# BoifZ/VDN-NeRF

Hardware: AMD Instinct MI355X
Metric: rays/sec (512-ray batch, 128 samples/ray) (higher is better)
Workload: dtype bf16; 1 GPU; training step of womsk_white (hierarchical sampling + render forward + backward + gradient all-reduce + Adam): SDF 8x256 + colour 4x256 + NeRF 8x256, 512 rays x (64 coarse + 64 importance + 32 outside) per GPU per step; pixels uniform over the full 800 x 800 frame; samples that enter the loss through exact zeros are skipped: 81 % of the foreground and 56 % of the background points evaluated; rays_per_gpu=512, samples_per_ray=128, outside_samples=32, parallelism=dp1, allreduce_bytes=5636348, background_points_evaluated_last_step=45590, background_points_total=81920, foreground_points_evaluated_last_step=52986, foreground_points_total=65536

## Files before the change

include/vdn_render.h:

```cpp
#ifndef VDN_RENDER_H
#define VDN_RENDER_H
#include <stdint.h>

#ifdef __cplusplus
extern "C" {
#endif

#define VDN_ABI_VERSION 28

int vdn_abi_version(void);

typedef struct {
    const float* g;
    const float* v;
    float* w_eff;
    float* inv_norm;
    int32_t rows, cols;
} VdnWeightNormDesc;
int vdn_weightnorm_materialize(const VdnWeightNormDesc* descs_dev, int n_layers, int max_rows, void* stream);

typedef struct {
    const float* src;
    const float* bias;
    const int32_t* kmap;
    const int32_t* nmap;
    char* dst;
    int64_t row_stride, col_stride;
    int32_t n0;
    int32_t k_pad;
    float scale;
    int32_t fmt;
    int32_t kt_begin;
    int32_t kt_count;
    int32_t write_bias;
    float bias_scale;
    const float* tail;
    int32_t tail_off;
    int32_t tail_n;
    int32_t tail_stride;
} VdnChunkDesc;
int vdn_build_images(const VdnChunkDesc* descs_dev, int n_chunks, void* stream);

int vdn_posenc(const float* in, float* out, int64_t P, int32_t d, int32_t n_freqs, void* stream);

typedef struct {
    const char* blob;
    const float* pts;
    const float* rays_o;
    const float* rays_d;
    const float* z;
    int32_t n_per_ray;
    int32_t z_ld;
    int32_t sdf_ld;
    int32_t P;
    float scale;
    float* sdf;
    void* feat;
    float* normals;
    void* S;
    const float* w8row;
    void* H;
    void* V;
    void* PE;
    const int32_t* active_idx;
    const int32_t* n_active;
    float* U_pe;
    int32_t tail_row0, tail_max_rows;
    int32_t cold_start;
} VdnSdfArgs;
int vdn_sdf_mlp_fwd_f32(int mode, const VdnSdfArgs* args_host, void* stream);
int vdn_sdf_mlp_fwd_bf16(int mode, const VdnSdfArgs* args_host, void* stream);
int vdn_sdf_fwd_tail_bf16(const VdnSdfArgs* args_host, void* stream);

typedef struct {
    const char* blob;
    const float* rays_o;
    const float* rays_d;
    const float* z;
    const float* normals;
    const void* feat;
    const float* pts;
    const float* dirs;
    float* out;
    void* save_h;
    void* save_small;
    int32_t n_per_ray;
    int32_t P;
    int32_t d_out;
    int32_t squeeze_out;
    const int32_t* active_idx;
    const int32_t* n_active;
    const float* extra;
    void* save_extra;
} VdnRenderNetArgs;
int vdn_rendernet_fwd_f32(const VdnRenderNetArgs* args_host, void* stream);
int vdn_rendernet_fwd_bf16(const VdnRenderNetArgs* args_host, void* stream);

typedef struct {
    const char* blob;
    const float* rays_o;
    const float* rays_d;
    const float* z;
    const float* pts4;
    const float* dirs;
    float* density;
    float* rgb;
    float* feat;
    void* save_h;
    void* save_pe;
    void* save_feature;
    void* save_vpe;
    void* save_hv;
    int32_t n_per_ray;
    int32_t P;
    const int32_t* active_idx;
    const int32_t* n_active;
} VdnNerfArgs;
int vdn_nerf_mlp_fwd_f32(const VdnNerfArgs* args_host, void* stream);
int vdn_nerf_mlp_fwd_bf16(const VdnNerfArgs* args_host, void* stream);


typedef struct {
    const float* near;
    const float* far;
    const float* lin_samples;
    const float* lin_outside;
    const float* out_lower;
    const float* out_upper;
    const float* t_rand;
    const float* t_rand_out;
    float* z;
    float* z_out;
    int32_t B, n_samples, n_outside, z_ld;
} VdnCoarseArgs;
int vdn_coarse_z(const VdnCoarseArgs* args_host, void* stream);

typedef struct {
    const float* rays_o;
    const float* rays_d;
    const float* z;
    const float* sdf;
    const float* u;
    float* new_z;
    float inv_s;
    int32_t B, M, ld, n_imp;
    const float* weights;
    int32_t w_ld, _pad;
} VdnUpsampleArgs;
int vdn_upsample_round(const VdnUpsampleArgs* args_host, void* stream);

typedef struct {
    const float* z;
    const float* sdf;
    const float* new_z;
    const float* new_sdf;
    float* z_out;
    float* sdf_out;
    int32_t B, M, K, ld, ld_out;
} VdnMergeArgs;
int vdn_merge_sorted(const VdnMergeArgs* args_host, void* stream);
int vdn_merge_upsample(const VdnMergeArgs* merge_host, const VdnUpsampleArgs* upsample_host, void* stream);
int vdn_sdf_upsample_bf16(const VdnSdfArgs* sdf_host, const VdnUpsampleArgs* upsample_host, void* stream);
int vdn_sdf_merge_upsample_bf16(const VdnSdfArgs* sdf_host, const VdnMergeArgs* merge_host, const VdnUpsampleArgs* upsample_host, void* stream);

typedef struct {
    const float* z;
    float* dists;
    float* mid_z;
    float sample_dist;
    int32_t B, n, ld;
} VdnSectionArgs;
int vdn_sections(const VdnSectionArgs* args_host, void* stream);

typedef struct {
    const float* rays_o;
    const float* rays_d;
    const float* sdf;
    const float* normals;
    const float* dists;
    const float* mid_z;
    const float* color;
    const float* feat;
    const float* variance;
    const float* bg_density;
    const float* bg_rgb;
    const float* bg_feat;
    const float* bg_dists;
    const float* background_rgb;
    float cos_anneal_ratio;
    int32_t B, N, T, feat_ch;
    float* weights;
    float* alpha_out;
    float* cdf;
    float* inside_sphere;
    float* color_out;
    float* feat_out;
    float* weight_sum;
    float* weight_max;
    float* s_val;
    float* eik_partial;
    float* eik_out;
    const float* cos_anneal_dev;
} VdnCompositeArgs;
int vdn_alpha_composite_fwd(const VdnCompositeArgs* args_host, void* stream);
int vdn_feat_composite(const VdnCompositeArgs* args_host, void* stream);

int vdn_shade_fused_f32(const VdnSdfArgs* sdf_host, const VdnRenderNetArgs* color_host, const VdnCompositeArgs* comp_host,
                        int32_t* ticket, void* stream);
int vdn_sdf_color_train_bf16(const VdnSdfArgs* sdf_host, const void* color_blob, int32_t squeeze_out, void* col_h, void* col_small,
                             float* col_out, void* stream);
int vdn_shade_fused_bf16(const VdnSdfArgs* sdf_host, const void* color_blob, int32_t squeeze_out, const VdnCompositeArgs* comp_host,
                         int32_t* ticket, void* stream);

typedef struct {
    const float* rays_o;
    const float* rays_d;
    const float* mid_z;
    const float* normals;
    int32_t B, N;
    float* eik_partial;
    float* eik_out;
} VdnEikonalArgs;
int vdn_eikonal_terms(const VdnEikonalArgs* args_host, void* stream);


typedef struct {
    const char* blob;
    const float* g_out;
    const float* out;
    const void* save_h;
    void* delta_out;
    void* delta_h;
    void* d_feat;
    float* d_normals;
    int32_t acc_feat;
    int32_t acc_normals;
    int32_t P;
    int32_t d_out;
    int32_t squeeze_out;
    const int32_t* active_idx;
    const int32_t* n_active;
    const float* dirs; const float* rays_d;
    int32_t n_per_ray;
    int32_t acc_pts;
    float* d_pts;
    float* d_dirs;
    float* d_extra;
} VdnRenderNetBwdArgs;
int vdn_rendernet_bwd_f32(const VdnRenderNetBwdArgs* args_host, void* stream);
int vdn_rendernet_bwd_bf16(const VdnRenderNetBwdArgs* args_host, void* stream);

typedef struct {
    const char* blob;
    const float* g_density;
    const float* g_rgb;
    const float* g_feat;
    const void* save_h;
    const void* save_hv;
    void* delta_o;
    void* delta_v;
    void* delta_head;
    void* delta_h;
    int32_t P;
    const int32_t* active_idx;
    const int32_t* n_active;
    const float* rays_o; const float* rays_d; const float* z;
    int32_t n_per_ray;
    float* d_pts;
    float* d_dirs;
} VdnNerfBwdArgs;
int vdn_nerf_mlp_bwd_f32(const VdnNerfBwdArgs* args_host, void* stream);
int vdn_nerf_mlp_bwd_bf16(const VdnNerfBwdArgs* args_host, void* stream);
typedef struct {
    const float* pts4;
    const float* dirs;
    float* d_pts4;
    float* d_dirs;
    int32_t accumulate;
} VdnNerfInputGradArgs;
int vdn_nerf_mlp_bwd_input_f32(const VdnNerfBwdArgs* args_host, const VdnNerfInputGradArgs* in_host, void* stream);
int vdn_nerf_mlp_bwd_input_bf16(const VdnNerfBwdArgs* args_host, const VdnNerfInputGradArgs* in_host, void* stream);

typedef struct {
    const char* blob;
    const float* pts;
    const float* rays_o;
    const float* rays_d;
    const float* z;
    int32_t n_per_ray;
    int32_t z_ld;
    int32_t P;
    float scale;
    const float* g_normals;
    const void* S;
    const void* V;
    void* UB;
    void* EX;
    int32_t s_from_h;
    const int32_t* active_idx;
    const int32_t* n_active;
} VdnSdfRbarArgs;
int vdn_sdf_bwd_rbar_f32(const VdnSdfRbarArgs* args_host, void* stream);
int vdn_sdf_bwd_rbar_bf16(const VdnSdfRbarArgs* args_host, void* stream);

typedef struct {
    const char* blob;
    const float* g_sdf;
    const void* g_feat;
    const void* S;
    const void* EX;
    void* AB;
    int32_t P;
    float scale;
    int32_t s_from_h;
    const int32_t* active_idx;
    const int32_t* n_active;
    const float* pts; const float* rays_o; const float* rays_d; const float* z;
    int32_t n_per_ray, z_ld;
    const float* g_normals;
    const float* U_pe;
    int32_t acc_pts;
    float* d_pts;
} VdnSdfFbarArgs;
int vdn_sdf_bwd_fbar_f32(const VdnSdfFbarArgs* args_host, void* stream);
int vdn_sdf_bwd_fbar_bf16(const VdnSdfFbarArgs* args_host, void* stream);
int vdn_sdf_bwd_split_bf16(const VdnSdfRbarArgs* rbar_host, const VdnSdfFbarArgs* fbar_host, void* stream);


typedef struct {
    const void* A1; const void* B1;
    const void* A2; const void* B2;
    int32_t lda1, ldb1, lda2, ldb2;
    int32_t P;
    int32_t m_tiles, n_tiles;
    int32_t splits;
    int32_t wg_begin;
    int32_t _pad;
    float* slab;
    float* colsum;
    const int32_t* P_dev;
} VdnDwDesc;
int vdn_dw_gemm_f32(const VdnDwDesc* descs_dev, int n_desc, int total_wgs, void* stream);
int vdn_dw_gemm_bf16(const VdnDwDesc* descs_dev, int n_desc, int total_wgs, void* stream);
int vdn_dw_entry_wgs_f32(int m_tiles, int n_tiles, int splits);
int vdn_dw_entry_wgs_bf16(int m_tiles, int n_tiles, int splits);

typedef struct {
    const float* slab; const float* colsum;
    const int32_t* rmap; const int32_t* cmap;
    float* target; float* btarget;
    int64_t t_stride;
    int32_t splits, M, N;
    int32_t accumulate;
    float scale, bscale;
    const float* xsum;
    int32_t xsplits, xM, xrow;
    float xscale;
} VdnDwFinalizeDesc;
int vdn_dw_finalize(const VdnDwFinalizeDesc* descs_dev, int n_desc, int max_M, int phase, void* stream);

typedef struct {
    const float* g; const float* v; const float* inv_norm; const float* dw_eff;
    float* dg; float* dv;
    int32_t rows, cols;
} VdnWeightNormBwdDesc;
int vdn_weightnorm_bwd(const VdnWeightNormBwdDesc* descs_dev, int n_layers, int max_rows, void* stream);

typedef struct {
    const float* rays_o; const float* rays_d;
    const float* sdf; const float* normals; const float* dists; const float* mid_z;
    const float* color; const float* feat; const float* variance;
    const float* bg_density; const float* bg_rgb; const float* bg_feat; const float* bg_dists;
    const float* background_rgb;
    float cos_anneal_ratio;
    int32_t B, N, T, feat_ch;
    const float* alpha;
    const float* weights;
    const float* eik;
    const float* g_color;
    const float* g_feat;
    const float* g_weights;
    const float* g_eik;
    const float* g_cdf;
    float* d_sdf;
    float* d_normals;
    float* d_color;
    float* d_feat;
    float* d_bg_density;
    float* d_bg_rgb;
    float* d_bg_feat;
    float* d_var_partial;
    float* d_variance;
    float* d_dists;
    float* d_bg_dists;
    float* d_dir_cos;
    float* feat_scratch;
    const float* cos_anneal_dev;
} VdnCompositeBwdArgs;
int vdn_alpha_composite_bwd(const VdnCompositeBwdArgs* args_host, void* stream);

int vdn_composite_train(const VdnCompositeArgs* fwd_host, const VdnCompositeBwdArgs* bwd_host, const float* true_rgb, float* g_color,
                        const int32_t* fg_count, float igr_weight, float grad_scale, void* stream);
int vdn_eikonal_reduce(const float* eik_partial, int32_t B, float* eik_out, void* stream);
int vdn_composite_fwd_train(const VdnCompositeArgs* fwd_host, const float* gt_feats, float* g_feats, float depth_weight, float grad_scale, void* stream);
int vdn_composite_bwd_train(const VdnCompositeBwdArgs* bwd_host, const float* color_out, const float* true_rgb, float* g_color,
                            const int32_t* fg_count, float igr_weight, float grad_scale, void* stream);

typedef struct {
    const float* rays_d;
    const float* mid_z;
    const float* bg_mid;
    const float* d_pts;
    const float* d_dirs;
    const float* d_dists;
    const float* d_dir_cos;
    const float* d_bg_pts;
    const float* d_bg_dirs;
    const float* d_bg_dists;
    int32_t B, N, T;
    float* d_rays_o;
    float* d_rays_d;
    float* d_z;
    float* d_z_out;
} VdnRayAdjointArgs;
int vdn_ray_adjoint(const VdnRayAdjointArgs* args_host, void* stream);

typedef struct {
    const float* color;
    const float* true_rgb;
    const float* mask;
    const float* feats;
    const float* gt_feats;
    const float* weights;
    const float* eik;
    float igr_weight, mask_weight, depth_weight, grad_scale;
    int32_t B, T, C, _pad;
    float* g_color;
    float* g_feats;
    float* g_weights;
    float* g_eik;
    float* out_scalars;
} VdnLossArgs;
int vdn_loss_fwd_bwd(const VdnLossArgs* args_host, void* stream);

int vdn_adam_step(float* param, const float* grad, float* exp_avg, float* exp_avg_sq, int64_t n,
                  float lr, float beta1, float beta2, float eps, int32_t step, void* stream);
int vdn_adam_step_ranges(float* param, const float* grad, float* exp_avg, float* exp_avg_sq, int64_t begin0, int64_t end0,
                         int64_t begin1, int64_t end1, float lr, float beta1, float beta2, float eps, int32_t step, void* stream);

typedef struct {
    const float* pixels_x;
    const float* pixels_y;
    const float* intrinsic_inv;
    const float* pose;
    const float* image;
    const float* mask;
    const float* feats;
    float* out;
    float* near;
    float* far;
    int32_t B, H, W, C, mask_ch, out_ld;
} VdnGenRaysArgs;
int vdn_gen_rays(const VdnGenRaysArgs* args_host, void* stream);

typedef struct {
    const float* rays_o;
    const float* rays_d;
    const float* mid_z;
    int32_t B, N, T;
    int32_t* active_idx;
    int32_t* n_active;
    int32_t* ray_counts;
} VdnBackgroundActiveArgs;
int vdn_background_active(const VdnBackgroundActiveArgs* args_host, void* stream);

typedef struct {
    const float* rays_o;
    const float* rays_d;
    const float* mid_z;
    int32_t B, N;
    float radius;
    int32_t complement;
    int32_t* active_idx;
    int32_t* n_active;
    int32_t* ray_counts;
} VdnForegroundActiveArgs;

typedef struct {
    const float* rays_o; const float* rays_d;
    float* z;
    const float* new_z;
    int32_t M_old, _pad;
    const float* z_out;
    float* z_feed;
    int32_t B, N, T, z_ld;
    float sample_dist, fg_radius;
    float* dists; float* mid_z;
    float* bg_dists; float* bg_mid;
    int32_t* fg_active_idx; int32_t* fg_n_active; int32_t* fg_ray_counts;
    int32_t* bg_active_idx; int32_t* bg_n_active; int32_t* bg_ray_counts;
} VdnTrainPrepArgs;
int vdn_train_prep(const VdnTrainPrepArgs* args_host, void* stream);
int vdn_foreground_active(const VdnForegroundActiveArgs* args_host, void* stream);

typedef struct {
    const float* u;
    float threshold;
    int32_t R;
    int32_t* counts;
    const int64_t* offsets;
    float* tri_pos;
    int64_t* tri_key;
} VdnMeshArgs;
int vdn_mesh_count(const VdnMeshArgs* args_host, void* stream);
int vdn_mesh_emit(const VdnMeshArgs* args_host, void* stream);

typedef struct {
    const float* u;
    double isovalue;
    int32_t R;
    uint8_t* cube_case;
    int32_t* n_verts;
    int32_t* n_tris;
    const int64_t* vert_offsets;
    const int64_t* tri_offsets;
    double* vertices;
    int64_t* triangles;
} VdnMeshMcArgs;
int vdn_mesh_mc_count(const VdnMeshMcArgs* args_host, void* stream);
int vdn_mesh_mc_emit(const VdnMeshMcArgs* args_host, void* stream);


typedef struct {
    const float* pixels_x;
    const float* pixels_y;
    const float* intrinsic_inv;
    const float* r;
    const float* t;
    const float* init_c2w;
    const float* image;
    const float* mask;
    const float* feats;
    float* out;
    float* near;
    float* far;
    int32_t B, H, W, C, mask_ch, out_ld;
} VdnGenRaysPoseArgs;
int vdn_gen_rays_pose(const VdnGenRaysPoseArgs* args_host, void* stream);

typedef struct {
    const float* pixels_x;
    const float* pixels_y;
    const float* intrinsic_inv;
    const float* r;
    const float* t;
    const float* init_c2w;
    const float* d_rays_o;
    const float* d_rays_d;
    const float* d_z;
    const float* lin_samples;
    const float* d_z_out;
    const float* z_out;
    float* grad_r;
    float* grad_t;
    double* scratch;
    int32_t B, N, O, n_samples, n_importance, cam, n_cams, _pad;
} VdnPoseAdjointArgs;
int vdn_pose_adjoint(const VdnPoseAdjointArgs* args_host, void* stream);
#ifdef __cplusplus
}
#endif
#endif
```

vdn-nerf_amd/csrc/k_nerf_bwd.h:

```cpp
#pragma once
#include <type_traits>
#include "mlp_engine.h"
#include "vdn_kernels.h"

namespace vdn {

template <class P, bool DPT, bool EXPL>
__global__ __launch_bounds__(P::kWaves * 64, P::kMinWavesPerEU) void nerf_bwd_kernel(NerfBwdArgs a, NerfInputGradArgs in) {
    using ST = typename P::store_t;
    constexpr int kSlot = P::stride(9);
    extern __shared__ __attribute__((aligned(16))) char smem[];
    WStream<P::kWaves, kSlot> ws;
    const bool want_pts = EXPL || a.d_pts != nullptr;
    ws.init(a.blob, smem, want_pts ? 83 : 80);
    const int lane = ws.lane, c = lane & 31, h = lane >> 5;
    const long n_rows = a.active_idx != nullptr ? (long)*a.n_active : (long)a.P;
    if ((long)blockIdx.x * P::kWaves * 32 >= n_rows) return;
    ws.warm_issue((n_rows + P::kWaves * 32 - 1) / (P::kWaves * 32), 256 * P::kMinWavesPerEU);
    warm_code_issue((std::is_same<P, BF16>::value) ? kWarmCodeNerfBwd : 0, (n_rows + P::kWaves * 32 - 1) / (P::kWaves * 32), 256 * P::kMinWavesPerEU, ws.warm_dump());
    const long p_raw = ((long)blockIdx.x * P::kWaves + ws.wave) * 32 + c;
    const bool ok = p_raw < n_rows;
    const long p = ok ? p_raw : n_rows - 1;
    const long pd = a.active_idx != nullptr ? (long)a.active_idx[p] : p;
    const long PS = P::plane(a.P, 256);
    constexpr int KO = DPT ? 4 : 1;
    constexpr int LDO = DPT ? 128 : 32;
    const ST* save_h = reinterpret_cast<const ST*>(a.save_h);
    const ST* save_hv = reinterpret_cast<const ST*>(a.save_hv);
    ST* delta_o = reinterpret_cast<ST*>(a.delta_o);
    ST* delta_v = reinterpret_cast<ST*>(a.delta_v);
    ST* delta_head = reinterpret_cast<ST*>(a.delta_head);
    ST* delta_h = reinterpret_cast<ST*>(a.delta_h);

    float x4[4] = {0.0f, 0.0f, 0.0f, 0.0f}, dir[3] = {0.0f, 0.0f, 0.0f}, pw[3] = {0.0f, 0.0f, 0.0f}, nrm = 1.0f;
    float dx4[4] = {0.0f, 0.0f, 0.0f, 0.0f}, ddir[3] = {0.0f, 0.0f, 0.0f};
    if (EXPL) {
#pragma unroll
        for (int d = 0; d < 4; ++d) x4[d] = in.pts4[pd * 4 + d];
#pragma unroll
        for (int d = 0; d < 3; ++d) dir[d] = in.dirs[pd * 3 + d];
    } else if (want_pts) {
        const long r = pd / a.n_per_ray;
        const float z = a.z[pd];
#pragma unroll
        for (int d = 0; d < 3; ++d) {
            dir[d] = a.rays_d[r * 3 + d];
            pw[d] = a.rays_o[r * 3 + d] + dir[d] * z;
        }
        nrm = sqrtf(pw[0] * pw[0] + pw[1] * pw[1] + pw[2] * pw[2]);
        const float rr = fminf(fmaxf(nrm, 1.0f), 1e10f);
#pragma unroll
        for (int d = 0; d < 3; ++d) x4[d] = pw[d] / rr;
        x4[3] = 1.0f / rr;
    }
    typename P::template Act<9> X;
    typename P::template Act<8> Y;
    {
        float g3[3];
#pragma unroll
        for (int d = 0; d < 3; ++d) g3[d] = a.g_rgb[pd * 3 + d];
        const f32x16 t16 = vals_tile<3>(g3, h, 0);
        X.set(0, t16);
        P::store_tile(delta_o, p, LDO, 0, h, t16, ok);
        if constexpr (DPT) {
#pragma unroll
            for (int kt = 0; kt < 3; ++kt) {
                const f32x16 g = F32::load_tile(a.g_feat, pd, 96, kt, h);
                X.set(kt + 1, g);
                P::store_tile(delta_o, p, LDO, kt + 1, h, g, ok);
            }
        }
    }
    auto ldH = [&](int l) VDN_INL { return [=](int nt) VDN_INL { return P::load_tile(save_h + l * PS, p, 256, nt, h); }; };
    auto mask_store = [&](auto& D, ST* dst, int ld) VDN_INL {
        return [&D, dst, ld, p, ok, h](int nt, const f32x16& acc, const f32x16& hv) VDN_INL {
            f32x16 o;
#pragma unroll
            for (int t = 0; t < 16; ++t) o[t] = hv[t] > 0.0f ? acc[t] : 0.0f;
            D.set(nt, o);
            P::store_tile(dst, p, ld, nt, h, o, ok);
        };
    };
    ws.all_issue = __any(ok);
    warm_l2_wait();
    ws.start();
    dense<P, KO, 4, false>(ws, X, 0, [&](int nt) VDN_INL { return P::load_tile(save_hv, p, 128, nt, h); },
                               mask_store(Y, delta_v, 128), 4);
    dense<P, 4, 9, false>(ws, Y, 0, NoPre{}, [&](int nt, const f32x16& acc, int) VDN_INL {
        if (nt < 8) {
            X.set(nt, acc);
            P::store_tile(delta_head, p, 288, nt, h, acc, ok);
        } else if (want_pts) {
            pe_adjoint_tile<3, 4, 0, P::kAccurateTrig>(acc, h, dir, ddir);
        }
    });
    {
        float g1[1] = {a.g_density[pd]};
        const f32x16 t16 = vals_tile<1>(g1, h, 0);
        X.set(8, t16);
        P::store_tile(delta_head, p, 288, 8, h, t16, ok);
    }
    dense<P, 9, 8, false, kBwdPrefetch>(ws, X, 0, ldH(7), mask_store(Y, delta_h + 7 * PS, 256), P::kTileOps, P::kTileOps);
    dense<P, 8, 8, false, kBwdPrefetch>(ws, Y, 0, ldH(6), mask_store(X, delta_h + 6 * PS, 256), P::kTileOps, P::kTileOps);
    dense<P, 8, 8, false, kBwdPrefetch>(ws, X, 0, ldH(5), mask_store(Y, delta_h + 5 * PS, 256), P::kTileOps, P::kTileOps);
    dense<P, 8, 11, false>(ws, Y, 0,
        [&](int nt) VDN_INL { return nt >= 3 ? P::load_tile(save_h + 4 * PS, p, 256, nt - 3, h) : f32x16{}; },
        [&](int nt, const f32x16& acc, const f32x16& hv) VDN_INL {
            if (nt >= 3) {
                f32x16 o;
#pragma unroll
                for (int t = 0; t < 16; ++t) o[t] = hv[t] > 0.0f ? acc[t] : 0.0f;
                X.set(nt - 3, o);
                P::store_tile(delta_h + 4 * PS, p, 256, nt - 3, h, o, ok);
            } else if (want_pts) {
                if (nt == 0) pe_adjoint_tile<4, 10, 0, P::kAccurateTrig>(acc, h, x4, dx4);
                else if (nt == 1) pe_adjoint_tile<4, 10, 1, P::kAccurateTrig>(acc, h, x4, dx4);
                else pe_adjoint_tile<4, 10, 2, P::kAccurateTrig>(acc, h, x4, dx4);
            }
        });
    dense<P, 8, 8, false, kBwdPrefetch>(ws, X, 0, ldH(3), mask_store(Y, delta_h + 3 * PS, 256), P::kTileOps, P::kTileOps);
    dense<P, 8, 8, false, kBwdPrefetch>(ws, Y, 0, ldH(2), mask_store(X, delta_h + 2 * PS, 256), P::kTileOps, P::kTileOps);
    dense<P, 8, 8, false, kBwdPrefetch>(ws, X, 0, ldH(1), mask_store(Y, delta_h + 1 * PS, 256), P::kTileOps, P::kTileOps);
    dense<P, 8, 8, false, kBwdPrefetch>(ws, Y, 0, ldH(0), mask_store(X, delta_h + 0 * PS, 256), P::kTileOps, P::kTileOps);
    if (want_pts) {
        dense<P, 8, 3, false>(ws, X, 0, NoPre{}, [&](int nt, const f32x16& acc, int) VDN_INL {
            if (nt == 0) pe_adjoint_tile<4, 10, 0, P::kAccurateTrig>(acc, h, x4, dx4);
            else if (nt == 1) pe_adjoint_tile<4, 10, 1, P::kAccurateTrig>(acc, h, x4, dx4);
            else pe_adjoint_tile<4, 10, 2, P::kAccurateTrig>(acc, h, x4, dx4);
        });
        if (EXPL) {
            if (ok && h == 0) {
#pragma unroll
                for (int d = 0; d < 4; ++d) in.d_pts4[pd * 4 + d] = (in.accumulate ? in.d_pts4[pd * 4 + d] : 0.0f) + dx4[d];
#pragma unroll
                for (int d = 0; d < 3; ++d) in.d_dirs[pd * 3 + d] = (in.accumulate ? in.d_dirs[pd * 3 + d] : 0.0f) + ddir[d];
            }
            return;
        }
        if (ok && h == 0) {
            const bool free_r = nrm >= 1.0f && nrm <= 1e10f;
            const float rr = fminf(fmaxf(nrm, 1.0f), 1e10f);
            const float pu = pw[0] * dx4[0] + pw[1] * dx4[1] + pw[2] * dx4[2];
#pragma unroll
            for (int d = 0; d < 3; ++d) {
                float v = dx4[d] / rr;
                if (free_r) v -= pw[d] * (pu / (rr * rr * rr) + dx4[3] / (rr * rr * rr));
                a.d_pts[pd * 3 + d] = v;
                a.d_dirs[pd * 3 + d] = ddir[d];
            }
        }
    }
}

template <class P, bool EXPL>
int launch_nerf_bwd_impl(const VdnNerfBwdArgs* args, const NerfInputGradArgs& in, void* stream_) {
    hipStream_t stream = (hipStream_t)stream_;
    const int ppw = P::kWaves * 32;
    const int grid = (args->P + ppw - 1) / ppw;
    const size_t lds = 3 * P::stride(9);
    static bool once = (allow_big_lds(nerf_bwd_kernel<P, false, EXPL>, lds), allow_big_lds(nerf_bwd_kernel<P, true, EXPL>, lds), true);
    (void)once;
    if (args->g_feat != nullptr)
        hipLaunchKernelGGL((nerf_bwd_kernel<P, true, EXPL>), dim3(grid), dim3(P::kWaves * 64), lds, stream, *args, in);
    else
        hipLaunchKernelGGL((nerf_bwd_kernel<P, false, EXPL>), dim3(grid), dim3(P::kWaves * 64), lds, stream, *args, in);
    return (int)hipGetLastError();
}

inline bool nerf_bwd_args_ok(const VdnNerfBwdArgs* args) {
    return args && args->P > 0 && args->blob && args->g_density && args->g_rgb && args->save_h && args->save_hv &&
           args->delta_o && args->delta_v && args->delta_head && args->delta_h;
}

template <class P>
int launch_nerf_bwd(const VdnNerfBwdArgs* args, void* stream) {
    if (!nerf_bwd_args_ok(args)) return -1;
    if (args->d_pts && (!args->d_dirs || !args->rays_o || !args->rays_d || !args->z || args->n_per_ray <= 0)) return -2;
    return launch_nerf_bwd_impl<P, false>(args, NerfInputGradArgs{}, stream);
}

template <class P>
int launch_nerf_bwd_input(const VdnNerfBwdArgs* args, const VdnNerfInputGradArgs* in, void* stream) {
    if (!nerf_bwd_args_ok(args)) return -1;
    if (!in || !in->pts4 || !in->dirs || !in->d_pts4 || !in->d_dirs) return -2;
    if (args->d_pts || args->d_dirs) return -3;
    return launch_nerf_bwd_impl<P, true>(args, *in, stream);
}

}
```

vdn-nerf_amd/csrc/k_nerf_fwd.h:

```cpp
#pragma once
#include "mlp_engine.h"
#include "vdn_kernels.h"

namespace vdn {

template <class P, bool DPT>
__global__ __launch_bounds__(P::kWaves * 64, P::kMinWavesPerEU) void nerf_fwd_kernel(NerfArgs a) {
    using ST = typename P::store_t;
    constexpr int kSlot = P::stride(11);
    extern __shared__ __attribute__((aligned(16))) char smem[];
    WStream<P::kWaves, kSlot> ws;
    ws.init(a.blob, smem, 64 + 9 + 4 + (DPT ? 4 : 1));
    const int lane = ws.lane, c = lane & 31, h = lane >> 5;
    const long n_rows = a.active_idx != nullptr ? (long)*a.n_active : (long)a.P;
    if ((long)blockIdx.x * P::kWaves * 32 >= n_rows) return;
    if (a.save_h != nullptr) ws.warm((n_rows + P::kWaves * 32 - 1) / (P::kWaves * 32), 256 * P::kMinWavesPerEU);
    const long q_raw = ((long)blockIdx.x * P::kWaves + ws.wave) * 32 + c;
    const bool ok = q_raw < n_rows;
    const long q = ok ? q_raw : n_rows - 1;
    const long p = a.active_idx != nullptr ? (long)a.active_idx[q] : q;
    const long r = p / a.n_per_ray;
    ST* save_h = reinterpret_cast<ST*>(a.save_h);
    const long PS = P::plane(a.P, 256);

    float dir[3], p4[4];
#pragma unroll
    for (int d = 0; d < 3; ++d) dir[d] = a.dirs ? a.dirs[p * 3 + d] : a.rays_d[r * 3 + d];
    if (a.pts4 != nullptr) {
#pragma unroll
        for (int d = 0; d < 4; ++d) p4[d] = a.pts4[p * 4 + d];
    } else {
        const float z = a.z[p];
        float q[3];
        float n2 = 0.0f;
#pragma unroll
        for (int d = 0; d < 3; ++d) {
            q[d] = a.rays_o[r * 3 + d] + a.rays_d[r * 3 + d] * z;
            n2 += q[d] * q[d];
        }
        const float rr = fminf(fmaxf(sqrtf(n2), 1.0f), 1e10f);
#pragma unroll
        for (int d = 0; d < 3; ++d) p4[d] = q[d] / rr;
        p4[3] = 1.0f / rr;
    }
    typename P::template Act<11> X;
    typename P::template Act<9> Y;
    auto put_pe = [&](bool save) VDN_INL {
        float pe[84];
        posenc<4, 10, P::kAccurateTrig>(p4, pe);
#pragma unroll
        for (int kt = 0; kt < 3; ++kt) {
            const f32x16 t16 = vals_tile<84>(pe, h, kt);
            X.set(kt, t16);
            if (save && a.save_pe != nullptr) P::store_tile(reinterpret_cast<ST*>(a.save_pe), q, 96, kt, h, t16, ok);
        }
    };
    auto relu_into = [&](auto& D, int t0, ST* save, int ld) VDN_INL {
        return [&D, t0, save, ld, q, ok, h](int nt, const f32x16& acc, int) VDN_INL {
            f32x16 o;
#pragma unroll
            for (int t = 0; t < 16; ++t) o[t] = relu0(acc[t]);
            D.set(t0 + nt, o);
            if (save != nullptr) P::store_tile(save, q, ld, nt, h, o, ok);
        };
    };
    auto sv = [&](int l) VDN_INL { return save_h ? save_h + l * PS : (ST*)nullptr; };
    const int est = save_h != nullptr ? P::kTileOps : 0;
    ws.all_issue = __any(ok);
    put_pe(true);
    ws.start();
    dense<P, 3, 8, true>(ws, X, 0, NoPre{}, relu_into(Y, 0, sv(0), 256), est);
    dense<P, 8, 8, true>(ws, Y, 0, NoPre{}, relu_into(X, 0, sv(1), 256), est);
    dense<P, 8, 8, true>(ws, X, 0, NoPre{}, relu_into(Y, 0, sv(2), 256), est);
    dense<P, 8, 8, true>(ws, Y, 0, NoPre{}, relu_into(X, 0, sv(3), 256), est);
    dense<P, 8, 8, true>(ws, X, 0, NoPre{}, relu_into(Y, 0, sv(4), 256), est);
#pragma unroll
    for (int kt = 0; kt < 8; ++kt) X.copy_tile(3 + kt, Y, kt);
    put_pe(false);
    dense<P, 11, 8, true>(ws, X, 0, NoPre{}, relu_into(Y, 0, sv(5), 256), est);
    dense<P, 8, 8, true>(ws, Y, 0, NoPre{}, relu_into(X, 0, sv(6), 256), est);
    dense<P, 8, 8, true>(ws, X, 0, NoPre{}, relu_into(Y, 0, sv(7), 256), est);
    dense<P, 8, 9, true>(ws, Y, 0, NoPre{}, [&](int nt, const f32x16& acc, int) VDN_INL {
        if (nt < 8) {
            X.set(nt, acc);
            if (a.save_feature != nullptr) P::store_tile(reinterpret_cast<ST*>(a.save_feature), q, 256, nt, h, acc, ok);
        } else {
            if (ok && h == 0) a.density[p] = acc[0];
        }
    });
    {
        float pe[27];
        posenc<3, 4, P::kAccurateTrig>(dir, pe);
        const f32x16 t16 = vals_tile<27>(pe, h, 0);
        X.set(8, t16);
        if (a.save_vpe != nullptr) P::store_tile(reinterpret_cast<ST*>(a.save_vpe), q, 32, 0, h, t16, ok);
    }
    dense<P, 9, 4, true>(ws, X, 0, NoPre{}, relu_into(Y, 0, reinterpret_cast<ST*>(a.save_hv), 128));
    dense<P, 4, DPT ? 4 : 1, true>(ws, Y, 0, NoPre{}, [&](int nt, const f32x16& acc, int) VDN_INL {
        if (nt == 0) {
            if (ok && h == 0) {
                a.rgb[p * 3 + 0] = acc[0];
                a.rgb[p * 3 + 1] = acc[1];
                a.rgb[p * 3 + 2] = acc[2];
            }
        } else {
            F32::store_tile(a.feat, p, 96, nt - 1, h, acc, ok);
        }
    });
}

template <class P>
int launch_nerf_fwd(const VdnNerfArgs* args, void* stream_) {
    hipStream_t stream = (hipStream_t)stream_;
    if (args == nullptr || args->P <= 0 || !args->blob || !args->density || !args->rgb || args->n_per_ray <= 0) return -1;
    if (!args->pts4 && (!args->rays_o || !args->rays_d || !args->z)) return -1;
    if (!args->dirs && !args->rays_d) return -1;
    const int ppw = P::kWaves * 32;
    const int grid = (args->P + ppw - 1) / ppw;
    const size_t lds = 3 * P::stride(11);
    static bool once = (allow_big_lds(nerf_fwd_kernel<P, false>, lds), allow_big_lds(nerf_fwd_kernel<P, true>, lds), true);
    (void)once;
    if (args->feat != nullptr)
        hipLaunchKernelGGL((nerf_fwd_kernel<P, true>), dim3(grid), dim3(P::kWaves * 64), lds, stream, *args);
    else
        hipLaunchKernelGGL((nerf_fwd_kernel<P, false>), dim3(grid), dim3(P::kWaves * 64), lds, stream, *args);
    return (int)hipGetLastError();
}

}
```

vdn-nerf_amd/csrc/k_nerf_fwd2.h:

```cpp
#pragma once
#include "mlp_flow.h"
#include "vdn_kernels.h"

namespace vdn {

template <bool DPT, bool SAVE>
struct NerfFwdProg {
    static constexpr int total = 64 + 9 + 4 + (DPT ? 4 : 1);
    static constexpr int kt(int c) {
        if (c < 0 || c >= total) return 0;
        if (c < 8) return 3;
        if (c < 40) return 8;
        if (c < 48) return 11;
        if (c < 73) return 8;
        if (c < 77) return 9;
        return 4;
    }
    static constexpr bool bias(int c) { return c >= 0 && c < total; }
    static constexpr int loads(int) { return 0; }
    static constexpr bool drained(int c) { return c == 39; }
    static constexpr int stores(int c) {
        if (!SAVE || c < 0 || c >= total) return 0;
        if (c < 64) return BF16::kTileOps;
        if (c < 72) return BF16::kTileOps;
        if (c < 73) return 0;
        if (c < 77) return BF16::kTileOps;
        return 0;
    }
};

#ifndef VDN_NERF_FWD_ST_MODE
#define VDN_NERF_FWD_ST_MODE VDN_PLANE_ST_MODE
#endif
template <bool DPT, bool SAVE>
__global__ __launch_bounds__(256, 2) void nerf_fwd2_kernel(NerfArgs a) {
    constexpr int kSt = VDN_NERF_FWD_ST_MODE;
    using P = BF16;
    using ST = unsigned short;
    using PG = NerfFwdProg<DPT, SAVE>;
    constexpr int kSlot = P::stride(11);
    extern __shared__ __attribute__((aligned(16))) char smem[];
    flow::Pipe<4, kSlot, 3, 2> pp;
    pp.init(a.blob, smem);
    const int lane = pp.lane, c = lane & 31, h = lane >> 5;
    const long n_rows = a.active_idx != nullptr ? (long)*a.n_active : (long)a.P;
    if ((long)blockIdx.x * 4 * 32 >= n_rows) return;
    char* const wdump = pp.warm_dump();
    if constexpr (SAVE) warm_l2_issue(a.blob, PG::total * kSlot, (n_rows + 127) / 128, 512, wdump);
    warm_code_issue(SAVE ? kWarmCodeNerfFwd2 : 0, (n_rows + 127) / 128, 512, wdump);
    const long q_raw = ((long)blockIdx.x * 4 + pp.wave) * 32 + c;
    const bool ok = q_raw < n_rows;
    const long q = ok ? q_raw : n_rows - 1;
    const long p = a.active_idx != nullptr ? (long)a.active_idx[q] : q;
    const long r = p / a.n_per_ray;
    ST* save_h = reinterpret_cast<ST*>(a.save_h);
    const long PS = P::plane(a.P, 256);

    float dir[3], p4[4];
#pragma unroll
    for (int d = 0; d < 3; ++d) dir[d] = a.dirs ? a.dirs[p * 3 + d] : a.rays_d[r * 3 + d];
    if (a.pts4 != nullptr) {
#pragma unroll
        for (int d = 0; d < 4; ++d) p4[d] = a.pts4[p * 4 + d];
    } else {
        const float z = a.z[p];
        float qq[3];
        float n2 = 0.0f;
#pragma unroll
        for (int d = 0; d < 3; ++d) {
            qq[d] = a.rays_o[r * 3 + d] + a.rays_d[r * 3 + d] * z;
            n2 += qq[d] * qq[d];
        }
        const float rr = fminf(fmaxf(sqrtf(n2), 1.0f), 1e10f);
#pragma unroll
        for (int d = 0; d < 3; ++d) p4[d] = qq[d] / rr;
        p4[3] = 1.0f / rr;
    }
    typename P::template Act<11> X;
    typename P::template Act<9> Y;
    bf16x8 pe_keep[6];
    {
        float pe[84];
        posenc<4, 10, false>(p4, pe);
#pragma unroll
        for (int kt = 0; kt < 3; ++kt) {
            const f32x16 t16 = vals_tile<84>(pe, h, kt);
            X.set(kt, t16);
            if constexpr (SAVE) {
                if (a.save_pe != nullptr) P::template store_tile<kSt>(reinterpret_cast<ST*>(a.save_pe), q, 96, kt, h, t16, true);
            }
        }
#pragma unroll
        for (int i = 0; i < 6; ++i) pe_keep[i] = X.r[i];
    }
    auto relu_into = [&](auto& D, int t0, ST* save, int ld) VDN_INL {
        return [&D, t0, save, ld, q, h](int nt, const f32x16& acc, int) VDN_INL {
            f32x16 o;
#pragma unroll
            for (int t = 0; t < 16; ++t) o[t] = relu0(acc[t]);
            D.set(t0 + nt, o);
            if constexpr (SAVE) P::template store_tile<kSt>(save, q, ld, nt, h, o, true);
        };
    };
    auto sv = [&](int l) VDN_INL { return save_h + l * PS; };
    warm_l2_wait();
    pp.template start<PG>();
    auto f0 = flow::flow_begin();
    auto f1 = flow::dense2<PG, 8>(f0, pp, X, flow::NoLoad{}, relu_into(Y, 0, sv(0), 256));
    auto f2 = flow::dense2<PG, 8>(f1, pp, Y, flow::NoLoad{}, relu_into(X, 0, sv(1), 256));
    auto f3 = flow::dense2<PG, 8>(f2, pp, X, flow::NoLoad{}, relu_into(Y, 0, sv(2), 256));
    auto f4 = flow::dense2<PG, 8>(f3, pp, Y, flow::NoLoad{}, relu_into(X, 0, sv(3), 256));
    auto f5 = flow::dense2<PG, 8>(f4, pp, X, flow::NoLoad{}, relu_into(Y, 0, sv(4), 256));
    auto f5d = flow::flow_drain(f5);
#pragma unroll
    for (int kt = 0; kt < 8; ++kt) X.copy_tile(3 + kt, Y, kt);
#pragma unroll
    for (int i = 0; i < 6; ++i) X.r[i] = pe_keep[i];
    auto f6 = flow::dense2<PG, 8>(f5d, pp, X, flow::NoLoad{}, relu_into(Y, 0, sv(5), 256));
    auto f7 = flow::dense2<PG, 8>(f6, pp, Y, flow::NoLoad{}, relu_into(X, 0, sv(6), 256));
    auto f8 = flow::dense2<PG, 8>(f7, pp, X, flow::NoLoad{}, relu_into(Y, 0, sv(7), 256));
    auto f9 = flow::dense2<PG, 9>(f8, pp, Y, flow::NoLoad{}, [&](int nt, const f32x16& acc, int) VDN_INL {
        if (nt < 8) {
            X.set(nt, acc);
            if constexpr (SAVE) {
                if (a.save_feature != nullptr) P::template store_tile<kSt>(reinterpret_cast<ST*>(a.save_feature), q, 256, nt, h, acc, true);
            }
        } else {
            if (ok && h == 0) a.density[p] = acc[0];
        }
    });
    {
        float pe[27];
        posenc<3, 4, false>(dir, pe);
        const f32x16 t16 = vals_tile<27>(pe, h, 0);
        X.set(8, t16);
        if constexpr (SAVE) {
            if (a.save_vpe != nullptr) P::template store_tile<kSt>(reinterpret_cast<ST*>(a.save_vpe), q, 32, 0, h, t16, true);
        }
    }
    auto f10 = flow::dense2<PG, 4, false>(f9, pp, X, flow::NoLoad{}, relu_into(Y, 0, reinterpret_cast<ST*>(a.save_hv), 128));
    auto f11 = flow::dense2<PG, DPT ? 4 : 1>(f10, pp, Y, flow::NoLoad{}, [&](int nt, const f32x16& acc, int) VDN_INL {
        if (nt == 0) {
            if (ok && h == 0) {
                a.rgb[p * 3 + 0] = acc[0];
                a.rgb[p * 3 + 1] = acc[1];
                a.rgb[p * 3 + 2] = acc[2];
            }
        } else {
            F32::store_tile(a.feat, p, 96, nt - 1, h, acc, ok);
        }
    });
    flow::flow_finish(f11);
}

inline int launch_nerf_fwd2(const VdnNerfArgs* args, void* stream_) {
    hipStream_t stream = (hipStream_t)stream_;
    if (args == nullptr || args->P <= 0 || !args->blob || !args->density || !args->rgb || args->n_per_ray <= 0) return -1;
    if (!args->pts4 && (!args->rays_o || !args->rays_d || !args->z)) return -1;
    if (!args->dirs && !args->rays_d) return -1;
    const bool save = args->save_h != nullptr;
    if (save && (!args->save_hv || !args->save_feature)) return -1;
    const int grid = (args->P + 127) / 128;
    const size_t lds = 3 * BF16::stride(11);
    static bool once = (allow_big_lds(nerf_fwd2_kernel<false, false>, lds), allow_big_lds(nerf_fwd2_kernel<true, false>, lds),
                        allow_big_lds(nerf_fwd2_kernel<false, true>, lds), allow_big_lds(nerf_fwd2_kernel<true, true>, lds), true);
    (void)once;
    const bool dpt = args->feat != nullptr;
#define VDN_L(D, S) hipLaunchKernelGGL((nerf_fwd2_kernel<D, S>), dim3(grid), dim3(256), lds, stream, *args)
    if (dpt) { if (save) VDN_L(true, true); else VDN_L(true, false); }
    else { if (save) VDN_L(false, true); else VDN_L(false, false); }
#undef VDN_L
    return (int)hipGetLastError();
}

}
```

vdn-nerf_amd/csrc/k_render_bwd.h:

```cpp
#pragma once
#include <type_traits>
#include "mlp_engine.h"
#include "vdn_kernels.h"

namespace vdn {

template <class P, int NT_OUT, int EX = 0>
__global__ __launch_bounds__(P::kWaves * 64, P::kMinWavesPerEU) void rendernet_bwd_kernel(RenderNetBwdArgs a) {
    using ST = typename P::store_t;
    constexpr int kSlot = P::stride(8);
    extern __shared__ __attribute__((aligned(16))) char smem[];
    WStream<P::kWaves, kSlot> ws;
    ws.init(a.blob, smem, 42 + EX);
    const int lane = ws.lane, c = lane & 31, h = lane >> 5;
    const WorkRow wr = work_row(a.active_idx, a.n_active, a.P, P::kWaves, ws.wave, c);
    if (wr.none) return;
    ws.warm_issue(wr.n_wg, 256 * P::kMinWavesPerEU);
    warm_code_issue((std::is_same<P, BF16>::value) ? kWarmCodeRenderBwd : 0, wr.n_wg, 256 * P::kMinWavesPerEU, ws.warm_dump());
    const bool ok = wr.ok;
    const long p = wr.row, pd = wr.point;
    const long PS = P::plane(a.P, 256);
    const ST* save_h = reinterpret_cast<const ST*>(a.save_h);
    ST* delta_h = reinterpret_cast<ST*>(a.delta_h);
    ST* delta_out = reinterpret_cast<ST*>(a.delta_out);
    ST* d_feat = reinterpret_cast<ST*>(a.d_feat);

    typename P::template Act<8> X, Y;
    if constexpr (NT_OUT == 1) {
        float dl[4];
#pragma unroll
        for (int j = 0; j < 4; ++j) {
            dl[j] = 0.0f;
            if (j < a.d_out) {
                const float o = a.out[pd * a.d_out + j], g = a.g_out[pd * a.d_out + j];
                dl[j] = a.squeeze_out ? g * o * (1.0f - o) : (o > 0.0f ? g : 0.0f);
            }
        }
        const f32x16 t16 = vals_tile<4>(dl, h, 0);
        X.set(0, t16);
        P::store_tile(delta_out, p, 32, 0, h, t16, ok);
    } else {
#pragma unroll
        for (int kt = 0; kt < 3; ++kt) {
            const f32x16 o = F32::load_tile(a.out, pd, 96, kt, h);
            const f32x16 g = F32::load_tile(a.g_out, pd, 96, kt, h);
            f32x16 dl;
#pragma unroll
            for (int t = 0; t < 16; ++t) dl[t] = a.squeeze_out ? g[t] * o[t] * (1.0f - o[t]) : (o[t] > 0.0f ? g[t] : 0.0f);
            X.set(kt, dl);
            P::store_tile(delta_out, p, 96, kt, h, dl, ok);
        }
    }
    auto ldH = [&](int l) VDN_INL { return [=](int nt) VDN_INL { return P::load_tile(save_h + l * PS, p, 256, nt, h); }; };
    auto mask_store = [&](auto& D, int l) VDN_INL {
        return [&D, l, delta_h, PS, p, ok, h](int nt, const f32x16& acc, const f32x16& hv) VDN_INL {
            f32x16 o;
#pragma unroll
            for (int t = 0; t < 16; ++t) o[t] = hv[t] > 0.0f ? acc[t] : 0.0f;
            D.set(nt, o);
            P::store_tile(delta_h + l * PS, p, 256, nt, h, o, ok);
        };
    };
    ws.all_issue = __any(ok);
    warm_l2_wait();
    ws.start();
    dense<P, NT_OUT, 8, false, kBwdPrefetch>(ws, X, 0, ldH(3), mask_store(Y, 3), P::kTileOps, P::kTileOps);
    dense<P, 8, 8, false, kBwdPrefetch>(ws, Y, 0, ldH(2), mask_store(X, 2), P::kTileOps, P::kTileOps);
    dense<P, 8, 8, false, kBwdPrefetch>(ws, X, 0, ldH(1), mask_store(Y, 1), P::kTileOps, P::kTileOps);
    dense<P, 8, 8, false, kBwdPrefetch>(ws, Y, 0, ldH(0), mask_store(X, 0), P::kTileOps, P::kTileOps);
    f32x16 SM[2];
    dense<P, 8, 10 + EX, false>(ws, X, 0, NoPre{}, [&](int nt, const f32x16& acc, int) VDN_INL {
        if (nt >= 10) {
            if constexpr (EX > 0) {
                f32x16 o = F32::load_tile(a.d_extra, pd, 32 * EX, nt - 10, h);
#pragma unroll
                for (int t = 0; t < 16; ++t) o[t] += acc[t];
                F32::store_tile(a.d_extra, pd, 32 * EX, nt - 10, h, o, ok);
            }
        } else if (nt < 8) {
            f32x16 o = acc;
            if (a.acc_feat) {
                const f32x16 prev = P::load_tile(d_feat, p, 256, nt, h);
#pragma unroll
                for (int t = 0; t < 16; ++t) o[t] += prev[t];
            }
            P::store_tile(d_feat, p, 256, nt, h, o, ok);
        } else {
            SM[nt - 8] = acc;
        }
    });
    float small[33];
    tiles_vals<33, 2>(SM, h, small);
    if (ok && h == 0) {
#pragma unroll
        for (int d = 0; d < 3; ++d) {
            const float prev = a.acc_normals ? a.d_normals[pd * 3 + d] : 0.0f;
            a.d_normals[pd * 3 + d] = prev + small[30 + d];
        }
        if (a.d_pts != nullptr) {
            const long r = pd / a.n_per_ray;
#pragma unroll
            for (int d = 0; d < 3; ++d) {
                const float dir = a.dirs ? a.dirs[pd * 3 + d] : a.rays_d[r * 3 + d];
                float g = small[3 + d];
#pragma unroll
                for (int k = 0; k < 4; ++k) {
                    const float f = (float)(1 << k);
                    float sn, co;
                    sincos_pe<P::kAccurateTrig>(dir * f, sn, co);
                    g += f * (co * small[3 + 3 + 6 * k + d] - sn * small[3 + 3 + 6 * k + 3 + d]);
                }
                const float pp = a.acc_pts ? a.d_pts[pd * 3 + d] : 0.0f;
                const float pg = a.acc_pts ? a.d_dirs[pd * 3 + d] : 0.0f;
                a.d_pts[pd * 3 + d] = pp + small[d];
                a.d_dirs[pd * 3 + d] = pg + g;
            }
        }
    }
}

template <class P>
int launch_rendernet_bwd(const VdnRenderNetBwdArgs* args, void* stream_) {
    hipStream_t stream = (hipStream_t)stream_;
    if (!args || args->P <= 0 || !args->blob || !args->g_out || !args->out || !args->save_h || !args->delta_out ||
        !args->delta_h || !args->d_feat || !args->d_normals) return -1;
    if (!(args->d_out == 96 || (args->d_out >= 1 && args->d_out <= 4))) return -2;
    if (args->d_pts && (!args->d_dirs || (!args->dirs && (!args->rays_d || args->n_per_ray <= 0)))) return -3;
    const int ppw = P::kWaves * 32;
    const int grid = (args->P + ppw - 1) / ppw;
    const size_t lds = 3 * P::stride(8);
    static bool once = (allow_big_lds(rendernet_bwd_kernel<P, 1>, lds), allow_big_lds(rendernet_bwd_kernel<P, 3>, lds),
                        allow_big_lds(rendernet_bwd_kernel<P, 1, 3>, lds), true);
    (void)once;
    if (args->d_extra != nullptr) {
        if (args->d_out == 96) return -4;
        hipLaunchKernelGGL((rendernet_bwd_kernel<P, 1, 3>), dim3(grid), dim3(P::kWaves * 64), lds, stream, *args);
        return (int)hipGetLastError();
    }
    if (args->d_out == 96)
        hipLaunchKernelGGL((rendernet_bwd_kernel<P, 3>), dim3(grid), dim3(P::kWaves * 64), lds, stream, *args);
    else
        hipLaunchKernelGGL((rendernet_bwd_kernel<P, 1>), dim3(grid), dim3(P::kWaves * 64), lds, stream, *args);
    return (int)hipGetLastError();
}

}
```

vdn-nerf_amd/csrc/k_render_fwd.h:

```cpp
#pragma once
#include <type_traits>
#include "mlp_engine.h"
#include "vdn_kernels.h"

namespace vdn {

template <class P, int NT_OUT, int EX = 0>
VDN_DEV void rendernet_fwd_body(const RenderNetArgs& a, char* smem) {
    using ST = typename P::store_t;
    constexpr int kSlot = P::stride(10 + EX);
    constexpr int kNSlot = 3 * kSlot > 160 * 1024 ? 2 : 3;
    WStream<P::kWaves, kSlot, kNSlot> ws;
    ws.init(a.blob, smem, 32 + NT_OUT);
    const int lane = ws.lane, c = lane & 31, h = lane >> 5;
    const WorkRow wr = work_row(a.active_idx, a.n_active, a.P, P::kWaves, ws.wave, c);
    if (wr.none) return;
    if (a.save_h != nullptr) ws.warm_issue(wr.n_wg, 256 * P::kMinWavesPerEU);
    warm_code_issue((a.save_h != nullptr && std::is_same<P, BF16>::value) ? kWarmCodeRenderFwd : 0, wr.n_wg, 256 * P::kMinWavesPerEU, ws.warm_dump());
    const bool ok = wr.ok;
    const long p = wr.row, pd = wr.point;
    const long r = pd / a.n_per_ray;
    const ST* feat = reinterpret_cast<const ST*>(a.feat);
    ST* save_h = reinterpret_cast<ST*>(a.save_h);
    ST* save_small = reinterpret_cast<ST*>(a.save_small);
    const long PS = P::plane(a.P, 256);

    typename P::template Act<10 + EX> X;
    typename P::template Act<8> Y;
#pragma unroll
    for (int kt = 0; kt < 8; ++kt) X.set(kt, P::load_tile(feat, p, 256, kt, h));
    if constexpr (EX > 0) {
#pragma unroll
        for (int kt = 0; kt < EX; ++kt) {
            const f32x16 t16 = F32::load_tile(a.extra, pd, 32 * EX, kt, h);
            X.set(10 + kt, t16);
            if (a.save_extra != nullptr) P::store_tile(reinterpret_cast<ST*>(a.save_extra), p, 32 * EX, kt, h, t16, ok);
        }
    }
    {
        float small[33];
        float dir[3];
        const float z = a.pts ? 0.0f : a.z[pd];
#pragma unroll
        for (int d = 0; d < 3; ++d) {
            dir[d] = a.dirs ? a.dirs[pd * 3 + d] : a.rays_d[r * 3 + d];
            small[d] = a.pts ? a.pts[pd * 3 + d] : a.rays_o[r * 3 + d] + a.rays_d[r * 3 + d] * z;
            small[30 + d] = a.normals[pd * 3 + d];
        }
        float pe[27];
        posenc<3, 4, P::kAccurateTrig>(dir, pe);
#pragma unroll
        for (int i = 0; i < 27; ++i) small[3 + i] = pe[i];
#pragma unroll
        for (int kt = 0; kt < 2; ++kt) {
            const f32x16 t16 = vals_tile<33>(small, h, kt);
            X.set(8 + kt, t16);
            if (save_small != nullptr) P::store_tile(save_small, p, 64, kt, h, t16, ok);
        }
    }
    auto relu_into = [&](auto& D, int l) VDN_INL {
        return [&D, l, save_h, PS, p, ok, h](int nt, const f32x16& acc, int) VDN_INL {
            f32x16 o;
#pragma unroll
            for (int t = 0; t < 16; ++t) o[t] = relu0(acc[t]);
            D.set(nt, o);
            if (save_h != nullptr) P::store_tile(save_h + l * PS, p, 256, nt, h, o, ok);
        };
    };
    const int est = save_h != nullptr ? P::kTileOps : 0;
    ws.all_issue = __any(ok);
    warm_l2_wait();
    ws.start();
    dense<P, 10 + EX, 8, true>(ws, X, 0, NoPre{}, relu_into(Y, 0), est);
    dense<P, 8, 8, true>(ws, Y, 0, NoPre{}, relu_into(X, 1), est);
    dense<P, 8, 8, true>(ws, X, 0, NoPre{}, relu_into(Y, 2), est);
    dense<P, 8, 8, true>(ws, Y, 0, NoPre{}, relu_into(X, 3), est);
    dense<P, 8, NT_OUT, true>(ws, X, 0, NoPre{}, [&](int nt, const f32x16& acc, int) VDN_INL {
        f32x16 o;
#pragma unroll
        for (int t = 0; t < 16; ++t) o[t] = a.squeeze_out ? sigmoidf_(acc[t]) : relu0(acc[t]);
        if constexpr (NT_OUT == 1) {
            if (ok && h == 0) {
                for (int j = 0; j < a.d_out && j < 4; ++j) a.out[pd * a.d_out + j] = o[j];
            }
        } else {
            F32::store_tile(a.out, pd, 96, nt, h, o, ok);
        }
    });
}

template <class P, int NT_OUT, int EX = 0>
__global__ __launch_bounds__(P::kWaves * 64, P::kMinWavesPerEU) void rendernet_fwd_kernel(RenderNetArgs a) {
    extern __shared__ __attribute__((aligned(16))) char smem[];
    rendernet_fwd_body<P, NT_OUT, EX>(a, smem);
}

template <class P>
int launch_rendernet_fwd(const VdnRenderNetArgs* args, void* stream_) {
    hipStream_t stream = (hipStream_t)stream_;
    if (args == nullptr || args->P <= 0 || !args->blob || !args->normals || !args->feat || !args->out || args->n_per_ray <= 0) return -1;
    if (!args->pts && (!args->rays_o || !args->rays_d || !args->z)) return -1;
    if (!args->dirs && !args->rays_d) return -1;
    if (!(args->d_out == 96 || (args->d_out >= 1 && args->d_out <= 4))) return -2;
    const int ppw = P::kWaves * 32;
    const int grid = (args->P + ppw - 1) / ppw;
    if (args->extra != nullptr) {
        if (args->d_out == 96) return -3;
        const size_t lds3 = (3 * P::stride(13) > 160 * 1024 ? 2 : 3) * P::stride(13);
        static bool once3 = (allow_big_lds(rendernet_fwd_kernel<P, 1, 3>, lds3), true);
        (void)once3;
        hipLaunchKernelGGL((rendernet_fwd_kernel<P, 1, 3>), dim3(grid), dim3(P::kWaves * 64), lds3, stream, *args);
        return (int)hipGetLastError();
    }
    const size_t lds = 3 * P::stride(10);
    static bool once = (allow_big_lds(rendernet_fwd_kernel<P, 1>, lds), allow_big_lds(rendernet_fwd_kernel<P, 3>, lds), true);
    (void)once;
    if (args->d_out == 96)
        hipLaunchKernelGGL((rendernet_fwd_kernel<P, 3>), dim3(grid), dim3(P::kWaves * 64), lds, stream, *args);
    else
        hipLaunchKernelGGL((rendernet_fwd_kernel<P, 1>), dim3(grid), dim3(P::kWaves * 64), lds, stream, *args);
    return (int)hipGetLastError();
}

}
```

vdn-nerf_amd/csrc/mlp_engine.h:

```cpp
#pragma once
#include <type_traits>
#include "vdn_common.h"

namespace vdn {

typedef __bf16 bf16x2_t __attribute__((ext_vector_type(2)));

VDN_DEV unsigned pack_bf16x2(float a, float b) {
    bf16x2_t v = {(__bf16)a, (__bf16)b};
    return __builtin_bit_cast(unsigned, v);
}
VDN_DEV float bf16_lo(unsigned u) { return __uint_as_float(u << 16); }
VDN_DEV float bf16_hi(unsigned u) { return __uint_as_float(u & 0xFFFF0000u); }


template <int NWAVES, int STRIDE, int NSLOT = 3>
struct WStream {
    static_assert(STRIDE % (1024 * NWAVES) == 0, "chunk stride must be a multiple of NWAVES KiB");
    static constexpr int DEPTH = NSLOT - 1;
    static constexpr int G = STRIDE / 1024 / NWAVES;
    const char* g;
    char* lds;
    int cur;
    int issued;
    int total;
    int wave, lane;
    bool all_issue;

    unsigned voff0, m0_wave;
    VDN_DEV void init(const char* blob, char* smem, int total_chunks) {
        g = blob;
        lds = smem;
        cur = -1;
        issued = 0;
        total = total_chunks;
        wave = threadIdx.x >> 6;
        lane = threadIdx.x & 63;
        all_issue = false;
        const int wv = __builtin_amdgcn_readfirstlane(wave);
        voff0 = lane * 16 + wv * (G * 1024) + 4096;
        m0_wave = __builtin_amdgcn_readfirstlane((unsigned)(size_t)smem + wv * (G * 1024) + 4096);
    }
    VDN_DEV char* warm_dump() const { return lds + (threadIdx.x >> 6) * (G * 1024); }
    VDN_DEV void warm(long n_wg, int resident) const { warm_l2(g, total * STRIDE, n_wg, resident, warm_dump()); }
    VDN_DEV void warm_issue(long n_wg, int resident) const { warm_l2_issue(g, total * STRIDE, n_wg, resident, warm_dump()); }
    VDN_DEV void issue_next() {
        const unsigned m0v = m0_wave + (unsigned)((issued % NSLOT) * STRIDE);
        static_for<G>([&](auto i_c) VDN_INL {
            constexpr int I = decltype(i_c)::value;
            if constexpr (I % 8 == 0) glds16_imm_m0<glds_imm(I)>(g, voff0 + glds_group_off(I), m0v + glds_group_off(I));
            else glds16_imm<glds_imm(I)>(g, voff0 + glds_group_off(I));
        });
        g += STRIDE;
        ++issued;
    }
    VDN_DEV void start() {
#pragma unroll
        for (int i = 0; i < DEPTH; ++i)
            if (issued < total) issue_next();
    }
    VDN_DEV const char* acquire(int younger = 0) {
        ++cur;
        if (!all_issue) younger = 0;
        const int ahead = min(issued - cur - 1, DEPTH - 1);
        wait_vm(younger + ahead * G);
#if !defined(VDN_ABLATE) || VDN_ABLATE != 3
        __builtin_amdgcn_s_barrier();
#endif
        asm volatile("" ::: "memory");
        if (issued < total) issue_next();
        return lds + (cur % NSLOT) * STRIDE;
    }
    static VDN_DEV void wait_vm(int n) {
        switch (n) {
#define VDN_W(k) case k: asm volatile("s_waitcnt vmcnt(" #k ")" ::: "memory"); break;
            VDN_W(1) VDN_W(2) VDN_W(3) VDN_W(4) VDN_W(5) VDN_W(6) VDN_W(7) VDN_W(8) VDN_W(9) VDN_W(10) VDN_W(11) VDN_W(12)
            VDN_W(13) VDN_W(14) VDN_W(15) VDN_W(16) VDN_W(17) VDN_W(18) VDN_W(19) VDN_W(20) VDN_W(21) VDN_W(22) VDN_W(23) VDN_W(24)
            VDN_W(25) VDN_W(26) VDN_W(27) VDN_W(28) VDN_W(29) VDN_W(30) VDN_W(31) VDN_W(32)
#undef VDN_W
            default: if (n > 32) { asm volatile("s_waitcnt vmcnt(32)" ::: "memory"); } else { asm volatile("s_waitcnt vmcnt(0)" ::: "memory"); } break;
        }
    }
};

VDN_DEV float sprime(float raw, int from_h) {
    if (from_h == 0) return raw;
    return 1.0f - __builtin_amdgcn_exp2f(from_h == 2 ? -raw : -144.26950408889634f * raw);
}

struct WorkRow {
    long row, point;
    bool ok, none;
    long n_wg;
};
VDN_DEV WorkRow work_row(const int32_t* active_idx, const int32_t* n_active, long P, int waves, int wave, int c) {
    WorkRow w;
    const long n_rows = active_idx != nullptr ? (long)*n_active : P;
    w.none = (long)blockIdx.x * waves * 32 >= n_rows;
    const long raw = ((long)blockIdx.x * waves + wave) * 32 + c;
    w.ok = raw < n_rows;
    w.row = w.ok ? raw : (n_rows > 0 ? n_rows - 1 : 0);
    w.point = active_idx != nullptr ? (long)active_idx[w.row] : w.row;
    w.n_wg = (n_rows + waves * 32 - 1) / (waves * 32);
    return w;
}

struct NoPre {
    VDN_DEV int operator()(int) const { return 0; }
};

struct F32 {
    static constexpr int kWaves = 4;
    static constexpr int kMinWavesPerEU = 1;
    static constexpr bool kAccurateTrig = true;
    static constexpr bool kOverlapEpilogue = false;
    static constexpr bool kDeriveS = false;
    static constexpr int chunk_bytes(int KT) { return KT * 4096 + 1024; }
    static constexpr int stride(int KTMAX) { return (chunk_bytes(KTMAX) + 4095) / 4096 * 4096; }
    static constexpr int kTileOps = 4;
    using store_t = float;

    template <int NT>
    struct Act {
        float r[NT * 16];
        VDN_DEV void set(int tile, const f32x16& v) {
#pragma unroll
            for (int t = 0; t < 16; ++t) {
                float x = v[t];
                asm volatile("" : "+v"(x));
                r[tile * 16 + t] = x;
            }
        }
        template <class A2>
        VDN_DEV void copy_tile(int dt, const A2& src, int st) {
#pragma unroll
            for (int t = 0; t < 16; ++t) r[dt * 16 + t] = src.r[st * 16 + t];
        }
    };

    template <int KT, bool BIAS, class ActT>
    static VDN_DEV f32x16 mma(const char* w, const ActT& X, int x0, int lane) {
        const int h = lane >> 5;
        const f32x4* wa = reinterpret_cast<const f32x4*>(w) + lane;
        f32x16 acc;
        if constexpr (BIAS) {
            const f32x4* bias = reinterpret_cast<const f32x4*>(w + KT * 4096);
#pragma unroll
            for (int q = 0; q < 4; ++q) {
                const f32x4 b = bias[2 * q + h];
                acc[4 * q + 0] = b[0]; acc[4 * q + 1] = b[1]; acc[4 * q + 2] = b[2]; acc[4 * q + 3] = b[3];
            }
        } else {
#pragma unroll
            for (int t = 0; t < 16; ++t) acc[t] = 0.0f;
        }
        static_for<KT * 4>([&](auto g_c) VDN_INL {
            constexpr int g = decltype(g_c)::value;
            const f32x4 a = wa[g * 64];
            acc = __builtin_amdgcn_mfma_f32_32x32x2f32(a[0], X.r[x0 * 16 + 4 * g + 0], acc, 0, 0, 0);
            acc = __builtin_amdgcn_mfma_f32_32x32x2f32(a[1], X.r[x0 * 16 + 4 * g + 1], acc, 0, 0, 0);
            acc = __builtin_amdgcn_mfma_f32_32x32x2f32(a[2], X.r[x0 * 16 + 4 * g + 2], acc, 0, 0, 0);
            acc = __builtin_amdgcn_mfma_f32_32x32x2f32(a[3], X.r[x0 * 16 + 4 * g + 3], acc, 0, 0, 0);
        });
        return acc;
    }

    static VDN_DEV long plane(long P, int ld) { return P * ld; }
    static VDN_DEV long rows(long P) { return P; }
    static VDN_DEV void store_tile(float* base, long row, int ld, int tile, int h, const f32x16& v, bool ok) {
        if (!ok) return;
        float* p = base + row * ld + tile * 32 + 4 * h;
#pragma unroll
        for (int q = 0; q < 4; ++q) {
            f32x4 o = {v[4 * q], v[4 * q + 1], v[4 * q + 2], v[4 * q + 3]};
            *reinterpret_cast<f32x4*>(p + 8 * q) = o;
        }
    }
    using raw_tile = f32x16;
    static VDN_DEV raw_tile load_raw(const float* base, long row, int ld, int tile, int h) { return load_tile(base, row, ld, tile, h); }
    static VDN_DEV f32x16 unpack(const raw_tile& r) { return r; }
    static VDN_DEV f32x16 load_tile(const float* base, long row, int ld, int tile, int h) {
        const float* p = base + row * ld + tile * 32 + 4 * h;
        f32x16 r;
#pragma unroll
        for (int q = 0; q < 4; ++q) {
            const f32x4 o = *reinterpret_cast<const f32x4*>(p + 8 * q);
            r[4 * q] = o[0]; r[4 * q + 1] = o[1]; r[4 * q + 2] = o[2]; r[4 * q + 3] = o[3];
        }
        return r;
    }
};

struct BF16 {
    static constexpr int kWaves = 4;
    static constexpr int kMinWavesPerEU = 2;
    static constexpr bool kAccurateTrig = false;
    static constexpr bool kOverlapEpilogue = true;
    static constexpr bool kDeriveS = true;
#ifndef VDN_SLOT_GROUP
#define VDN_SLOT_GROUP 2
#endif
    static constexpr int kSlotGroup = VDN_SLOT_GROUP;
    static constexpr int chunk_bytes(int KT) { return KT * 2048 + 1024; }
    static constexpr int stride(int KTMAX) { return (chunk_bytes(KTMAX) + 4095) / 4096 * 4096; }
    using store_t = unsigned short;

    template <int NT>
    struct Act {
        bf16x8 r[NT * 2];
        VDN_DEV void set(int tile, const f32x16& v) {
#pragma unroll
            for (int s = 0; s < 2; ++s) {
                typedef unsigned u32x4 __attribute__((ext_vector_type(4)));
                u32x4 pk;
#pragma unroll
                for (int j = 0; j < 4; ++j) {
                    unsigned x = pack_bf16x2(v[8 * s + 2 * j], v[8 * s + 2 * j + 1]);
                    asm volatile("" : "+v"(x));
                    pk[j] = x;
                }
                r[tile * 2 + s] = __builtin_bit_cast(bf16x8, pk);
            }
        }
        template <class A2>
        VDN_DEV void copy_tile(int dt, const A2& src, int st) {
            r[dt * 2] = src.r[st * 2];
            r[dt * 2 + 1] = src.r[st * 2 + 1];
        }
    };

    template <int KT, bool BIAS, class ActT>
    static VDN_DEV f32x16 mma(const char* w, const ActT& X, int x0, int lane) {
        const int h = lane >> 5;
        const bf16x8* wa = reinterpret_cast<const bf16x8*>(w) + lane;
        f32x16 acc;
        if constexpr (BIAS) {
            const f32x4* bias = reinterpret_cast<const f32x4*>(w + KT * 2048);
#pragma unroll
            for (int q = 0; q < 4; ++q) {
                const f32x4 b = bias[2 * q + h];
                acc[4 * q + 0] = b[0]; acc[4 * q + 1] = b[1]; acc[4 * q + 2] = b[2]; acc[4 * q + 3] = b[3];
            }
        } else {
#pragma unroll
            for (int t = 0; t < 16; ++t) acc[t] = 0.0f;
        }
#if defined(VDN_ABLATE) && VDN_ABLATE == 2
        (void)wa;
        return acc;
#endif
        constexpr int NS = KT * 2;
        constexpr int PRE = NS < 6 ? NS : 6;
        bf16x8 fr[NS];
        static_for<NS>([&](auto s_c) VDN_INL {
            constexpr int s = decltype(s_c)::value;
            fr[s] = wa[s * 64];
        });
        static_for<NS>([&](auto s_c) VDN_INL {
            constexpr int s = decltype(s_c)::value;
            acc = __builtin_amdgcn_mfma_f32_32x32x16_bf16(fr[s], X.r[x0 * 2 + s], acc, 0, 0, 0);
        });
        __builtin_amdgcn_sched_group_barrier(0x100, PRE + (BIAS ? 2 : 0), 0);
        static_for<NS - PRE>([&](auto) VDN_INL {
            __builtin_amdgcn_sched_group_barrier(0x008, 1, 0);
            __builtin_amdgcn_sched_group_barrier(0x100, 1, 0);
        });
        __builtin_amdgcn_sched_group_barrier(0x008, PRE, 0);
        return acc;
    }

    template <int KT, bool BIAS, class ActT, class Slot>
    static VDN_DEV f32x16 mma_slots(const char* w, const ActT& X, int x0, int lane, Slot&& slot) {
        const int h = lane >> 5;
        const bf16x8* wa = reinterpret_cast<const bf16x8*>(w) + lane;
        constexpr int NS = KT * 2;
        constexpr int PRE = NS < 6 ? NS : 6;
        f32x16 acc;
        bf16x8 fr[NS];
        static_for<PRE>([&](auto s_c) VDN_INL {
            constexpr int s = decltype(s_c)::value;
            fr[s] = wa[s * 64];
        });
        if constexpr (BIAS) {
            const f32x4* bias = reinterpret_cast<const f32x4*>(w + KT * 2048);
#pragma unroll
            for (int q = 0; q < 4; ++q) {
                const f32x4 b = bias[2 * q + h];
                acc[4 * q + 0] = b[0]; acc[4 * q + 1] = b[1]; acc[4 * q + 2] = b[2]; acc[4 * q + 3] = b[3];
            }
        } else {
#pragma unroll
            for (int t = 0; t < 16; ++t) acc[t] = 0.0f;
        }
        __builtin_amdgcn_sched_barrier(0);
        static_for<NS>([&](auto s_c) VDN_INL {
            constexpr int s = decltype(s_c)::value;
            acc = __builtin_amdgcn_mfma_f32_32x32x16_bf16(fr[s], X.r[x0 * 2 + s], acc, 0, 0, 0);
            if constexpr (s + PRE < NS) fr[s + PRE] = wa[(s + PRE) * 64];
            slot(s_c, std::integral_constant<int, NS>{});
            if constexpr ((s + 1) % kSlotGroup == 0 || s + 1 == NS) __builtin_amdgcn_sched_barrier(0);
        });
        return acc;
    }

    static constexpr int kTileOps = 2;
    static VDN_DEV long rows(long P) { return (P + 31) & ~31L; }
    static VDN_DEV long plane(long P, int ld) { return rows(P) * ld; }
    template <int MODE = VDN_PLANE_ST_MODE>
    static VDN_DEV void store_tile(unsigned short* base, long row, int ld, int tile, int h, const f32x16& v, bool ok) {
        if (!ok) return;
        unsigned short* p = base + (row >> 5) * (32L * ld) + tile * 1024 + h * 256 + (row & 31) * 8;
#pragma unroll
        for (int k = 0; k < 2; ++k) {
            uint4 o;
            o.x = pack_bf16x2(v[8 * k], v[8 * k + 1]);
            o.y = pack_bf16x2(v[8 * k + 2], v[8 * k + 3]);
            o.z = pack_bf16x2(v[8 * k + 4], v[8 * k + 5]);
            o.w = pack_bf16x2(v[8 * k + 6], v[8 * k + 7]);
            typedef unsigned wt_u32x4 __attribute__((ext_vector_type(4)));
            const wt_u32x4 ov = {o.x, o.y, o.z, o.w};
            if constexpr (MODE == 1) asm volatile("global_store_dwordx4 %0, %1, off sc1\n\ts_nop 1" ::"v"(p + 512 * k), "v"(ov) : "memory");
            else if constexpr (MODE == 2) asm volatile("global_store_dwordx4 %0, %1, off nt\n\ts_nop 1" ::"v"(p + 512 * k), "v"(ov) : "memory");
            else if constexpr (MODE == 3) asm volatile("global_store_dwordx4 %0, %1, off sc1 nt\n\ts_nop 1" ::"v"(p + 512 * k), "v"(ov) : "memory");
            else if constexpr (MODE == 4) { asm volatile("" ::"v"(p + 512 * k), "v"(ov)); }
            else *reinterpret_cast<uint4*>(p + 512 * k) = o;
        }
    }
    struct raw_tile { uint4 k[2]; };
    static VDN_DEV raw_tile load_raw(const unsigned short* base, long row, int ld, int tile, int h) {
        const unsigned short* p = base + (row >> 5) * (32L * ld) + tile * 1024 + h * 256 + (row & 31) * 8;
        raw_tile r;
#ifdef VDN_PLANE_LD_NT
        typedef unsigned nt_u32x4 __attribute__((ext_vector_type(4)));
        const nt_u32x4 a = __builtin_nontemporal_load(reinterpret_cast<const nt_u32x4*>(p));
        const nt_u32x4 b = __builtin_nontemporal_load(reinterpret_cast<const nt_u32x4*>(p + 512));
        r.k[0] = make_uint4(a[0], a[1], a[2], a[3]);
        r.k[1] = make_uint4(b[0], b[1], b[2], b[3]);
#else
        r.k[0] = *reinterpret_cast<const uint4*>(p);
        r.k[1] = *reinterpret_cast<const uint4*>(p + 512);
#endif
        return r;
    }
    static VDN_DEV f32x16 unpack(const raw_tile& t) {
        f32x16 r;
#pragma unroll
        for (int k = 0; k < 2; ++k) {
            const uint4 o = t.k[k];
            r[8 * k] = bf16_lo(o.x); r[8 * k + 1] = bf16_hi(o.x); r[8 * k + 2] = bf16_lo(o.y); r[8 * k + 3] = bf16_hi(o.y);
            r[8 * k + 4] = bf16_lo(o.z); r[8 * k + 5] = bf16_hi(o.z); r[8 * k + 6] = bf16_lo(o.w); r[8 * k + 7] = bf16_hi(o.w);
        }
        return r;
    }
    static VDN_DEV f32x16 load_tile(const unsigned short* base, long row, int ld, int tile, int h) {
        return unpack(load_raw(base, row, ld, tile, h));
    }
};

template <class ScratchT, class Elem, class Finish>
struct ElemEpi {
    using Scratch = ScratchT;
    Elem elem;
    Finish finish;
    template <class Aux>
    VDN_DEV void operator()(int nt, const f32x16& acc, const Aux& aux) const {
        Scratch sc;
#pragma unroll
        for (int t = 0; t < 16; ++t) elem(nt, t, acc[t], sc);
        finish(nt, sc, aux);
    }
};
template <class ScratchT, class Elem, class Finish>
VDN_DEV ElemEpi<ScratchT, Elem, Finish> elem_epi(Elem e, Finish f) { return {e, f}; }
template <class T> struct is_elem_epi : std::false_type {};
template <class S, class E, class F> struct is_elem_epi<ElemEpi<S, E, F>> : std::true_type {};

template <class P, int KT, int NT, bool BIAS, int PF = 1, class WS, class ActT, class Pre, class Epi>
VDN_DEV void dense(WS& ws, const ActT& X, int x0, Pre&& pre, Epi&& epi, int epi_stores = 0, int pre_loads = 0) {
    const int lane = ws.lane;
    using EpiT = std::remove_cv_t<std::remove_reference_t<Epi>>;
    if constexpr (P::kOverlapEpilogue && is_elem_epi<EpiT>::value) {
        f32x16 acc_prev;
        decltype(pre(0)) aux_prev{};
        static_for<NT + 1>([&](auto s_c) VDN_INL {
            constexpr int s = decltype(s_c)::value;
            typename EpiT::Scratch sc;
            if constexpr (s < NT) {
                constexpr int D = WS::DEPTH;
                constexpr int n_pre = s < D ? s : D;
                constexpr int n_epi = s <= D ? (s > 0 ? s - 1 : 0) : D;
                const int yg = n_pre * pre_loads + n_epi * epi_stores;
                const char* w = ws.acquire(yg);
                auto aux_cur = pre(s);
                const f32x16 acc_cur = P::template mma_slots<KT, BIAS>(w, X, x0, lane, [&](auto k_c, auto ns_c) VDN_INL {
                    if constexpr (s > 0) {
                        constexpr int k = decltype(k_c)::value, NS = decltype(ns_c)::value;
                        static_for<(k + 1) * 16 / NS - k * 16 / NS>([&](auto j_c) VDN_INL {
                            constexpr int t = k * 16 / NS + decltype(j_c)::value;
                            epi.elem(s - 1, t, acc_prev[t], sc);
                        });
                    }
                });
                if constexpr (s > 0) epi.finish(s - 1, sc, aux_prev);
                acc_prev = acc_cur;
                aux_prev = aux_cur;
            } else {
#pragma unroll
                for (int t = 0; t < 16; ++t) epi.elem(s - 1, t, acc_prev[t], sc);
                epi.finish(s - 1, sc, aux_prev);
            }
            __builtin_amdgcn_sched_barrier(0);
        });
        return;
    }
    using Aux = decltype(pre(0));
    Aux ring[PF];
    static_for<PF>([&](auto i_c) VDN_INL {
        constexpr int i = decltype(i_c)::value;
        if constexpr (i < NT) ring[i] = pre(i);
    });
    static_for<NT>([&](auto nt_c) VDN_INL {
        constexpr int nt = decltype(nt_c)::value;
        constexpr int n_steps = nt < WS::DEPTH ? nt : WS::DEPTH;
        constexpr int n_pre = [] { int n = 0; for (int j = nt - n_steps; j < nt; ++j) n += (j + PF < NT) ? 1 : 0; return n; }();
        const int yg = n_steps * epi_stores + n_pre * pre_loads;
        const char* w = ws.acquire(yg);
        Aux nxt{};
        if constexpr (nt + PF < NT) nxt = pre(nt + PF);
        const f32x16 acc = P::template mma<KT, BIAS>(w, X, x0, lane);
        epi(nt, acc, ring[nt % PF]);
        if constexpr (nt + PF < NT) ring[nt % PF] = nxt;
        __builtin_amdgcn_sched_barrier(0);
    });
}

#ifndef VDN_BWD_PF
#define VDN_BWD_PF 2
#endif
constexpr int kBwdPrefetch = VDN_BWD_PF;

template <int NF>
VDN_DEV f32x16 vals_tile(const float (&vals)[NF], int h, int tile) {
    f32x16 o;
#pragma unroll
    for (int t = 0; t < 16; ++t) {
        const int f0 = 32 * tile + (t & 3) + 8 * (t >> 2);
        const int f1 = f0 + 4;
        const float a = f0 < NF ? vals[f0 < NF ? f0 : 0] : 0.0f;
        const float b = f1 < NF ? vals[f1 < NF ? f1 : 0] : 0.0f;
        o[t] = h ? b : a;
    }
    return o;
}
template <int NF, int NT>
VDN_DEV void tiles_vals(const f32x16 (&T)[NT], int h, float (&vals)[NF]) {
#pragma unroll
    for (int tile = 0; tile < NT; ++tile) {
#pragma unroll
        for (int t = 0; t < 16; ++t) {
            const int f0 = 32 * tile + (t & 3) + 8 * (t >> 2);
            const int f1 = f0 + 4;
            const float mine = T[tile][t];
            const float other = __shfl_xor(mine, 32);
            if (f0 < NF) vals[f0 < NF ? f0 : 0] = h ? other : mine;
            if (f1 < NF) vals[f1 < NF ? f1 : 0] = h ? mine : other;
        }
    }
}

template <int D, int L, int T0, bool ACCURATE>
VDN_DEV void pe_adjoint_tile(const f32x16& tile, int h, const float (&x)[D], float (&dx)[D]) {
    float g[32];
    const f32x16 t1[1] = {tile};
    tiles_vals<32, 1>(t1, h, g);
#pragma unroll
    for (int j = 0; j < 32; ++j) {
        const int slot = 32 * T0 + j;
        if (slot >= D * (1 + 2 * L)) continue;
        if (slot < D) {
            dx[slot] += g[j];
        } else {
            const int k = (slot - D) / (2 * D), w = (slot - D) % (2 * D), d = w % D;
            const float f = (float)(1 << k);
            float sn, co;
            sincos_pe<ACCURATE>(x[d] * f, sn, co);
            dx[d] += w >= D ? -f * sn * g[j] : f * co * g[j];
        }
    }
}

}
```

vdn-nerf_amd/vdn_hip/layout.py:

```python
import torch


def pad32(P):
    return (P + 31) // 32 * 32


def rows(P, precision):
    return P if precision == "fp32" else pad32(P)


def to_pt32(x):
    P, ld = x.shape
    Pp = pad32(P)
    buf = torch.zeros(Pp, ld, dtype=torch.bfloat16, device=x.device)
    buf[:P] = x.to(torch.bfloat16)
    return buf.view(Pp // 32, 32, ld // 32, 2, 2, 2, 4).permute(0, 2, 3, 5, 1, 4, 6).contiguous().view(-1)


def from_pt32(buf, P, ld):
    Pp = pad32(P)
    x = buf.view(-1)[:Pp * ld].view(Pp // 32, ld // 32, 2, 2, 32, 2, 4).permute(0, 4, 1, 2, 5, 3, 6).contiguous().view(Pp, ld)
    return x[:P].float()


def col_offset_elems(col0, precision):
    if precision == "fp32":
        return col0
    assert col0 % 32 == 0
    return (col0 // 32) * 1024
```

vdn-nerf_amd/vdn_hip/train.py:

```python
import os

import numpy as np
import torch

from . import images, layout, lib

PTS_PER_SPLIT = int(os.environ.get("VDN_DW_SPLIT_PTS", "4096"))


def _pts_per_split(net, precision="bf16"):
    if precision == "fp32":
        dflt = "2048"
        return int(os.environ.get("VDN_DW_SPLIT_PTS_SDF" if net == "sdf" else "VDN_DW_SPLIT_PTS_REST", dflt))
    if net == "sdf":
        return int(os.environ.get("VDN_DW_SPLIT_PTS_SDF", os.environ.get("VDN_DW_SPLIT_PTS", "6144")))
    rest = os.environ.get("VDN_DW_SPLIT_PTS_REST", str(PTS_PER_SPLIT))
    return int(os.environ.get("VDN_DW_SPLIT_PTS_NERF" if net == "nerf" else "VDN_DW_SPLIT_PTS_HEADS", rest))


_stream = lib.stream_handle


_SHARED_STREAMS = {}


def shared_stream(dev, role):
    key = (torch.device(dev).index if torch.device(dev).index is not None else torch.cuda.current_device(), role)
    st = _SHARED_STREAMS.get(key)
    if st is None:
        st = _SHARED_STREAMS[key] = torch.cuda.Stream(device=dev)
    return st


class _Net:

    def __init__(self, module, dev, grad_views):
        self.module = module
        self.img = module._images()
        self.dweff = torch.zeros_like(self.img.weff)
        self.grads = {}
        for name, (g, v, b) in self.img.matrices.items():
            for t in (g, v, b):
                if t is not None:
                    self.grads[id(t)] = grad_views[id(t)]

    def dweff_view(self, name):
        v = self.img.matrices[name][1]
        o = self.img.w_off[name]
        return self.dweff[o:o + v.numel()].view(v.shape)

    def dw_target(self, name):
        g, v, b = self.img.matrices[name]
        return self.dweff_view(name) if g is not None else self.grads[id(v)]

    def bias_target(self, name):
        b = self.img.matrices[name][2]
        return None if b is None else self.grads[id(b)]



def _sl(t, l, ld=256):
    return (t, l * t.shape[1] * t.shape[2], 0, ld)


def _whole(t, c0=0):
    return (t, 0, c0, t.shape[1])


def sdf_dw_entries(H, V, PE, UB, AB, P, Pp, precision):
    ub_off, off = {}, 0
    for l, cols in enumerate((64, 256, 256, 256, 288, 256, 256, 256, 256)):
        ub_off[l] = (off, cols)
        off += Pp * cols
    ub = lambda l, c0=0: (UB, ub_off[l][0], c0, ub_off[l][1])
    ab = lambda l: (AB, 0, 0, 288) if l == 8 else (AB, Pp * 288 + (7 - l) * Pp * 256, 0, 256)
    maps = images.sdf_layer_maps()
    unit = 1.0 / images.SDF_UNIT if precision == "bf16" else 1.0
    maps = [(name, km, nm, sc * unit) for (name, km, nm, sc) in maps]
    ent = []
    for l, (name, km, nm, sc) in enumerate(maps):
        if l == 8:
            ent.append(dict(net="sdf", name=name, rmap=nm, cmap=km, scale=sc, A=ab(8), B=_sl(H, 7), bias=True, Pn=P))
            continue
        A, A2 = ab(l), _sl(V, l)
        if l == 0:
            ent.append(dict(net="sdf", name=name, rmap=nm, cmap=km, scale=sc, A=A, B=_whole(PE), A2=A2, B2=ub(0), bias=True, Pn=P))
        elif l == 4:
            ent.append(dict(net="sdf", name=name, rmap=nm, cmap=km[:224], scale=sc, A=A, B=_sl(H, 3), A2=A2, B2=ub(4), bias=True, Pn=P))
            ent.append(dict(net="sdf", name=name, rmap=nm, cmap=km[224:], scale=sc, A=A, B=_whole(PE), A2=A2, B2=ub(4, 224), bias=False, Pn=P))
        else:
            ent.append(dict(net="sdf", name=name, rmap=nm, cmap=km, scale=sc, A=A, B=_sl(H, l - 1), A2=A2, B2=ub(l), bias=True, Pn=P))
    ent.append(dict(net="sdf", name="lin8", rmap=images.ident_map(256), cmap=None, scale=1.0, A=ub(8), B=None, bias=False, Pn=P,
                    extra_row0=True))
    return ent


def rendering_dw_entries(net, km0, dh, dout, save_h, small, feat, extra, P, d_out):
    pad = 96 if d_out == 96 else 32
    I256 = images.ident_map(256)
    ent = [dict(net=net, name="lin0", rmap=I256, cmap=km0[:256], scale=1.0, A=_sl(dh, 0), B=_whole(feat), bias=True, Pn=P),
           dict(net=net, name="lin0", rmap=I256, cmap=km0[256:320], scale=1.0, A=_sl(dh, 0), B=_whole(small), bias=False, Pn=P)]
    if len(km0) > 320:
        ent.append(dict(net=net, name="lin0", rmap=I256, cmap=km0[320:], scale=1.0, A=_sl(dh, 0), B=_whole(extra), bias=False, Pn=P))
    for l in (1, 2, 3):
        ent.append(dict(net=net, name="lin%d" % l, rmap=I256, cmap=I256, scale=1.0, A=_sl(dh, l), B=_sl(save_h, l - 1), bias=True, Pn=P))
    ent.append(dict(net=net, name="lin4", rmap=images.ident_map(d_out, pad), cmap=I256, scale=1.0, A=_whole(dout), B=_sl(save_h, 3),
                    bias=True, Pn=P))
    return ent


def nerf_dw_entries(streams, dh, h, pe, dhead, dv, feature, vpe, do, hv, Q, with_dpt):
    km5, kmv = streams["_km5"], streams["_kmv"]
    I256 = images.ident_map(256)
    ent = [dict(net="nerf", name="pts_linears.0", rmap=I256, cmap=images.ident_map(84, 96), scale=1.0, A=_sl(dh, 0), B=_whole(pe), bias=True, Pn=Q)]
    for i in (1, 2, 3, 4, 6, 7):
        ent.append(dict(net="nerf", name="pts_linears.%d" % i, rmap=I256, cmap=I256, scale=1.0, A=_sl(dh, i), B=_sl(h, i - 1), bias=True, Pn=Q))
    ent.append(dict(net="nerf", name="pts_linears.5", rmap=I256, cmap=km5[:96], scale=1.0, A=_sl(dh, 5), B=_whole(pe), bias=True, Pn=Q))
    ent.append(dict(net="nerf", name="pts_linears.5", rmap=I256, cmap=km5[96:], scale=1.0, A=_sl(dh, 5), B=_sl(h, 4), bias=False, Pn=Q))
    ent.append(dict(net="nerf", name="feature_linear", rmap=I256, cmap=I256, scale=1.0, A=(dhead, 0, 0, 288), B=_sl(h, 7), bias=True, Pn=Q))
    ent.append(dict(net="nerf", name="alpha_linear", rmap=images.ident_map(1, 32), cmap=I256, scale=1.0, A=(dhead, 0, 256, 288), B=_sl(h, 7), bias=True, Pn=Q))
    ent.append(dict(net="nerf", name="views_linears.0", rmap=images.ident_map(128), cmap=kmv[:256], scale=1.0, A=_whole(dv), B=_whole(feature), bias=True, Pn=Q))
    ent.append(dict(net="nerf", name="views_linears.0", rmap=images.ident_map(128), cmap=kmv[256:], scale=1.0, A=_whole(dv), B=_whole(vpe), bias=False, Pn=Q))
    ldo = do.shape[1]
    ent.append(dict(net="nerf", name="rgb_linear", rmap=images.ident_map(3, 32), cmap=images.ident_map(128), scale=1.0, A=(do, 0, 0, ldo), B=_whole(hv), bias=True, Pn=Q))
    if with_dpt:
        ent.append(dict(net="nerf", name="dpt_linear", rmap=images.ident_map(96), cmap=images.ident_map(128), scale=1.0, A=(do, 0, 32, ldo), B=_whole(hv), bias=True, Pn=Q))
    return ent


def dw_layout(ent, precision):
    sfx = "_f32" if precision == "fp32" else "_bf16"
    all_maps, moff = [], 0
    slab_elems, cs_elems, wg = 0, 0, 0
    lay = []
    for e in ent:
        mt = len(e["rmap"]) // 32
        nt = 0 if e["cmap"] is None else len(e["cmap"]) // 32
        segs = 2 if e.get("A2") is not None else 1
        K = e["Pn"] * segs
        pps = _pts_per_split(e["net"], precision)
        splits = max(1, (K + pps - 1) // pps)
        if segs == 2:
            splits += splits % 2
        lay.append((mt, nt, splits, slab_elems, cs_elems, moff, wg))
        all_maps.append(np.asarray(e["rmap"], np.int32))
        moff += mt * 32
        if nt:
            all_maps.append(np.asarray(e["cmap"], np.int32))
            moff += nt * 32
        slab_elems += splits * mt * 32 * nt * 32
        cs_elems += splits * mt * 32
        wg += lib.call_value("vdn_dw_entry_wgs" + sfx, mt, nt, splits)
    return lay, all_maps, slab_elems, cs_elems, wg


def dw_tables(ent, lay, nets, precision, slab, colsum, maps, p_dev, sdf_scale):
    dw = np.zeros(len(ent), dtype=lib.struct_dtype("VdnDwDesc"))
    fin = np.zeros(len(ent), dtype=lib.struct_dtype("VdnDwFinalizeDesc"))
    P4 = lambda spec: spec[0].data_ptr() + spec[0].element_size() * (spec[1] + layout.col_offset_elems(spec[2], precision))
    for i, e in enumerate(ent):
        mt, nt, splits, so, co, mo, wg0 = lay[i]
        d = dw[i]
        d["A1"], d["lda1"] = P4(e["A"]), e["A"][3]
        if e["B"] is not None:
            d["B1"], d["ldb1"] = P4(e["B"]), e["B"][3]
        if e.get("A2") is not None:
            d["A2"], d["lda2"], d["B2"], d["ldb2"] = P4(e["A2"]), e["A2"][3], P4(e["B2"]), e["B2"][3]
        d["P"], d["m_tiles"], d["n_tiles"], d["splits"], d["wg_begin"] = e["Pn"], mt, nt, splits, wg0
        d["P_dev"] = p_dev[i]
        d["slab"] = slab.data_ptr() + 4 * so
        want_cs = e["bias"] or e.get("extra_row0")
        d["colsum"] = colsum.data_ptr() + 4 * co if want_cs else 0
        net = nets[e["net"]]
        fd = fin[i]
        fd["slab"], fd["colsum"] = d["slab"], d["colsum"]
        fd["rmap"] = maps.data_ptr() + 4 * mo
        fd["cmap"] = maps.data_ptr() + 4 * (mo + mt * 32)
        fd["splits"], fd["M"], fd["N"] = splits, mt * 32, nt * 32
        fd["scale"] = e["scale"]
        if e.get("extra_row0"):
            main = next(k for k, x in enumerate(ent) if x["net"] == e["net"] and x["name"] == e["name"] and not x.get("extra_row0"))
            fm = fin[main]
            fm["xsum"], fm["xsplits"], fm["xM"], fm["xrow"] = d["colsum"], splits, mt * 32, 0
            fm["xscale"] = 1.0 / sdf_scale
            fd["slab"], fd["colsum"] = 0, 0
        else:
            tgt = net.dw_target(e["name"])
            fd["target"], fd["t_stride"] = tgt.data_ptr(), tgt.shape[1]
            if e["bias"]:
                bt = net.bias_target(e["name"])
                fd["btarget"], fd["bscale"] = bt.data_ptr(), 1.0
    return dw, fin


def weightnorm_table(nets):
    rows = []
    for net in nets:
        for name, (g, v, b) in net.img.matrices.items():
            if g is not None:
                rows.append((g, v, net.img.inv_norm[net.img.r_off[name]:], net.dweff_view(name), net.grads[id(g)], net.grads[id(v)]))
    wn = np.zeros(len(rows), dtype=lib.struct_dtype("VdnWeightNormBwdDesc"))
    for i, (g, v, inv, dwe, dg, dv) in enumerate(rows):
        wn[i]["g"], wn[i]["v"], wn[i]["inv_norm"], wn[i]["dw_eff"] = g.data_ptr(), v.data_ptr(), inv.data_ptr(), dwe.data_ptr()
        wn[i]["dg"], wn[i]["dv"], wn[i]["rows"], wn[i]["cols"] = dg.data_ptr(), dv.data_ptr(), v.shape[0], v.shape[1]
    return wn, rows


class TrainEngine:
    def __init__(self, renderer, B, dev):
        self.r = renderer
        self.B, self.dev = B, dev
        S, I, O = renderer.n_samples, renderer.n_importance, renderer.n_outside
        self.N = S + I
        self.T = self.N + O
        self.P = B * self.N
        self.Q = B * self.T
        self.wdepth = renderer.depth_network is not None
        self.dbc = renderer.color_network.conf["d_feature"] == 352
        if self.dbc and not self.wdepth:
            raise ValueError("a d_feature = 352 colour network needs a depth_network (renderer.py:245-248)")
        use_side = os.environ.get("VDN_SIDE_STREAM", "1") == "1" and torch.device(dev).type == "cuda"
        self._side = shared_stream(dev, "side") if use_side else None
        self._ev_fork = torch.cuda.Event() if use_side else None
        self._ev_join = torch.cuda.Event() if use_side else None
        self._side2 = shared_stream(dev, "side2") if (use_side and renderer.depth_network is not None) else None
        self._ev_fork2 = torch.cuda.Event() if self._side2 is not None else None
        self._ev_join2 = torch.cuda.Event() if self._side2 is not None else None
        self._ev_heads = torch.cuda.Event() if use_side else None
        self._pending = False
        self._fused_keep = None
        self._fg_compact = self._bg_compact = False
        precs = {m.precision for m in (renderer.nerf, renderer.sdf_network, renderer.color_network, renderer.depth_network) if m is not None}
        if len(precs) != 1:
            raise ValueError("all networks of a renderer must share one precision, got %s" % sorted(precs))
        self.precision = precs.pop()
        self.sfx = "_f32" if self.precision == "fp32" else "_bf16"
        sdt = torch.float32 if self.precision == "fp32" else torch.bfloat16
        f = lambda *shape: torch.empty(*shape, dtype=torch.float32, device=dev)
        fs = lambda *shape: torch.empty(*shape, dtype=sdt, device=dev)
        P, Q, N, T = self.P, self.Q, self.N, self.T
        Pp, Qp = layout.rows(P, self.precision), layout.rows(Q, self.precision)
        self.Pp, self.Qp = Pp, Qp
        w = self.w = {}
        w["dists"] = f(B, N)
        fz = lambda *shape: torch.zeros(*shape, dtype=torch.float32, device=dev)
        slots, n_out = {}, 0
        for name, shape in (("color", (B, 3)), ("weights", (B, T)), ("eik", (3,)), ("feat_out", (B, 96) if self.wdepth else None),
                            ("cdf", (B, N)), ("normals", (P, 3)), ("inside", (B, N)), ("s_val", (B, 1)),
                            ("bg_mid", (B, T) if O > 0 else None), ("mid_z", (B, N)), ("wsum", (B, 1)), ("wmax", (B, 1))):
            if shape is not None:
                slots[name] = (n_out, shape)
                n_out += (int(np.prod(shape)) + 63) // 64 * 64
        self._out_arena, self._out_slots = fz(n_out), slots
        out = lambda name: self._out_arena[slots[name][0]:slots[name][0] + int(np.prod(slots[name][1]))].view(slots[name][1])
        w["sdf"], w["feat"], w["normals"], w["mid_z"] = fz(P), fs(Pp, 256), out("normals"), out("mid_z")
        w["fg_active"] = (torch.zeros(P, dtype=torch.int32, device=dev), torch.zeros(1, dtype=torch.int32, device=dev),
                          torch.zeros(B, dtype=torch.int32, device=dev))
        w["H"], w["V"], w["PE"] = fs(8, Pp, 256), fs(8, Pp, 256), fs(Pp, 64)
        if self.precision == "fp32":
            w["S"] = fs(8, Pp, 256)
        w["col_out"], w["col_h"], w["col_small"] = fz(P, 3), fs(4, Pp, 256), fs(Pp, 64)
        if self.wdepth:
            w["vdn_out"], w["vdn_h"], w["vdn_small"] = fz(P, 96), fs(4, Pp, 256), fs(Pp, 64)
        if self.dbc:
            w["col_extra"] = fs(Pp, 96)
        if O > 0:
            w["z_feed"], w["bg_dists"], w["bg_mid"] = f(B, T), f(B, T), out("bg_mid")
            w["bg_density"], w["bg_rgb"] = torch.zeros(Q, device=dev), torch.zeros(Q, 3, device=dev)
            w["bg_feat"] = torch.zeros(Q, 96, device=dev) if self.wdepth else None
            w["bg_active"] = (torch.zeros(Q, dtype=torch.int32, device=dev), torch.zeros(1, dtype=torch.int32, device=dev),
                              torch.zeros(B, dtype=torch.int32, device=dev))
            w["nf_h"], w["nf_pe"], w["nf_feature"], w["nf_vpe"], w["nf_hv"] = fs(8, Qp, 256), fs(Qp, 96), fs(Qp, 256), fs(Qp, 32), fs(Qp, 128)
        w["weights"], w["alpha"], w["cdf"], w["inside"] = out("weights"), f(B, T), out("cdf"), out("inside")
        w["color"], w["wsum"], w["wmax"], w["s_val"] = out("color"), out("wsum"), out("wmax"), out("s_val")
        w["eik_partial"], w["eik"] = f(B, 2), out("eik")
        w["feat_out"] = out("feat_out") if self.wdepth else None
        w["d_sdf"], w["d_normals"], w["d_color"], w["d_featvec"] = f(P), f(P, 3), f(P, 3), fs(Pp, 256)
        w["d_vdn"] = f(P, 96) if self.wdepth else None
        w["feat_scratch"] = f(B * (2 * T + N)) if self.wdepth else None
        w["d_var_partial"], w["d_variance"] = f(B), f(1)
        w["col_dout"], w["col_dh"] = fs(Pp, 32), fs(4, Pp, 256)
        if self.wdepth:
            w["vdn_dout"], w["vdn_dh"] = fs(Pp, 96), fs(4, Pp, 256)
        w["UB"], w["EX"], w["AB"] = fs(Pp * 2144), fs(8, Pp, 256), fs(Pp * 2336)
        if O > 0:
            w["d_bg_density"], w["d_bg_rgb"] = f(Q), f(Q, 3)
            w["d_bg_feat"] = f(Q, 96) if self.wdepth else None
            w["nf_do"], w["nf_dv"], w["nf_dhead"], w["nf_dh"] = fs(Qp, 128 if self.wdepth else 32), fs(Qp, 128), fs(Qp, 288), fs(8, Qp, 256)
        self.params = renderer._all_parameters()
        total = sum(p.numel() for p in self.params)
        self._grad_flat = torch.zeros(total, dtype=torch.float32, device=dev)
        views, off = {}, 0
        for p in self.params:
            views[id(p)] = self._grad_flat[off:off + p.numel()].view(p.shape)
            off += p.numel()
        self.grad_views = views
        self.nets = {"sdf": _Net(renderer.sdf_network, dev, views), "color": _Net(renderer.color_network, dev, views)}
        if self.wdepth:
            self.nets["vdn"] = _Net(renderer.depth_network, dev, views)
        if O > 0:
            self.nets["nerf"] = _Net(renderer.nerf, dev, views)
        self._build_dw_plan()

    def _build_dw_plan(self):
        w, P, Q = self.w, self.P, self.Q
        Pp, Qp, prec = self.Pp, self.Qp, self.precision
        ent = sdf_dw_entries(w["H"], w["V"], w["PE"], w["UB"], w["AB"], P, Pp, prec)
        ent += rendering_dw_entries("color", self.nets["color"].img.streams["fwd"][0].kmap, w["col_dh"], w["col_dout"], w["col_h"],
                                    w["col_small"], w["feat"], w.get("col_extra"), P, 3)
        if self.wdepth:
            ent += rendering_dw_entries("vdn", self.nets["vdn"].img.streams["fwd"][0].kmap, w["vdn_dh"], w["vdn_dout"], w["vdn_h"],
                                        w["vdn_small"], w["feat"], None, P, 96)
        if "nerf" in self.nets:
            ent += nerf_dw_entries(self.nets["nerf"].img.streams, w["nf_dh"], w["nf_h"], w["nf_pe"], w["nf_dhead"], w["nf_dv"],
                                   w["nf_feature"], w["nf_vpe"], w["nf_do"], w["nf_hv"], Q, self.wdepth)

        dev = self.dev
        n_sdf = sum(1 for e in ent if e["net"] == "sdf")
        assert all(e["net"] == "sdf" for e in ent[:n_sdf]) and all(e["net"] != "sdf" for e in ent[n_sdf:])
        lay, all_maps, slab_elems, cs_elems, wg = dw_layout(ent, prec)
        self.dw_total_wgs = wg
        self.maps = torch.from_numpy(np.concatenate(all_maps)).to(dev)
        self.slab = torch.empty(max(slab_elems, 1), dtype=torch.float32, device=dev)
        self.colsum = torch.empty(max(cs_elems, 1), dtype=torch.float32, device=dev)
        self.dw_list_kind = ["bg" if e["net"] == "nerf" else "fg" for e in ent]
        p_dev = [(w["bg_active"] if k == "bg" else w["fg_active"])[1].data_ptr() for k in self.dw_list_kind]
        dw, fin = dw_tables(ent, lay, self.nets, prec, self.slab, self.colsum, self.maps, p_dev, float(self.r.sdf_network.scale))
        self.dw_table = torch.from_numpy(dw.view(np.uint8)).to(dev)
        wg_sdf = int(dw[n_sdf]["wg_begin"]) if n_sdf < len(ent) else wg
        rest = dw[n_sdf:].copy()
        rest["wg_begin"] -= wg_sdf
        self.dw_groups = {"sdf": (self.dw_table, n_sdf, wg_sdf)}
        if len(rest):
            self.dw_groups["rest"] = (torch.from_numpy(rest.view(np.uint8)).to(dev), len(rest), wg - wg_sdf)
        n_heads_end = n_sdf + sum(1 for e in ent if e["net"] not in ("sdf", "nerf"))
        assert all(e["net"] == "nerf" for e in ent[n_heads_end:])
        sub_ranges = {"heads": (n_sdf, n_heads_end), "nerf": (n_heads_end, len(ent))}
        for gname, (lo, hi) in sub_ranges.items():
            if hi > lo:
                sub = dw[lo:hi].copy()
                wg_lo = int(dw[lo]["wg_begin"])
                wg_hi = int(dw[hi]["wg_begin"]) if hi < len(ent) else wg
                sub["wg_begin"] -= wg_lo
                self.dw_groups[gname] = (torch.from_numpy(sub.view(np.uint8)).to(dev), hi - lo, wg_hi - wg_lo)
        vfin = np.zeros(1, dtype=fin.dtype)
        self._var_map = torch.zeros(1, dtype=torch.int32, device=dev)
        vfin[0]["colsum"], vfin[0]["rmap"] = w["d_var_partial"].data_ptr(), self._var_map.data_ptr()
        vfin[0]["btarget"], vfin[0]["bscale"] = self.grad_views[id(self.r.deviation_network.variance)].data_ptr(), 1.0
        vfin[0]["splits"], vfin[0]["M"], vfin[0]["N"] = self.B, 1, 0
        fin_all = np.concatenate([fin, vfin])
        self.fin_table = torch.from_numpy(fin_all.view(np.uint8)).to(dev)
        self.fin_has_phase1 = bool((fin_all["accumulate"] != 0).any())
        self.n_fin = len(fin_all)
        self.n_dw = len(ent)
        self.fin_max_M = int(max(len(e["rmap"]) for e in ent))
        fg = {"sdf": np.concatenate([fin[:n_sdf], vfin]), "rest": fin[n_sdf:]}
        mm = {"sdf": ent[:n_sdf], "rest": ent[n_sdf:]}
        for gname, (lo, hi) in sub_ranges.items():
            fg[gname], mm[gname] = fin[lo:hi], ent[lo:hi]
        self.fin_groups = {k: (torch.from_numpy(v.view(np.uint8).copy()).to(dev), len(v), int(max(len(e["rmap"]) for e in mm[k])),
                               bool((v["accumulate"] != 0).any())) for k, v in fg.items() if len(v) and len(mm[k])}
        row_group = []
        for key, net in self.nets.items():
            for name, (g, v, b) in net.img.matrices.items():
                if g is not None:
                    row_group.append(("sdf",) if key == "sdf" else ("rest", "nerf" if key == "nerf" else "heads"))
        wn, rows = weightnorm_table(self.nets.values())
        self.wn_table = torch.from_numpy(wn.view(np.uint8).copy() if len(rows) else np.zeros(8, np.uint8)).to(dev)
        self.n_wn = len(rows)
        self.wn_max_rows = max([r[1].shape[0] for r in rows] + [1])
        self.wn_groups = {}
        for k in ("sdf", "rest", "heads", "nerf"):
            idx = [i for i, gk in enumerate(row_group) if k in gk]
            if idx:
                self.wn_groups[k] = (torch.from_numpy(wn[idx].view(np.uint8).copy()).to(dev), len(idx), max(rows[i][1].shape[0] for i in idx))
        self._param_ptrs = self._ptr_key()

    @property
    def grad_flat(self):
        if getattr(self, "join_hook", None) is not None:
            self.join_hook()
        return self._grad_flat

    def _ptr_key(self):
        return tuple(p.data_ptr() for net in self.nets.values() for p in lib.module_params(net.module))

    def _ray_workspaces(self):
        w, B, N, T, P, Q, dev = self.w, self.B, self.N, self.T, self.P, self.Q, self.dev
        if "U_pe" not in w:
            f = lambda *shape: torch.zeros(*shape, dtype=torch.float32, device=dev)
            w["U_pe"], w["d_pts"], w["d_dirs"] = f(P, 39), f(P, 3), f(P, 3)
            w["d_dists"], w["d_dir_cos"] = f(B, N), f(B, 3)
            w["d_rays_o"], w["d_rays_d"], w["d_z"] = f(B, 3), f(B, 3), f(B, N)
            if self.r.n_outside > 0:
                w["d_bg_pts"], w["d_bg_dirs"], w["d_bg_dists"], w["d_z_out"] = f(Q, 3), f(Q, 3), f(B, T), f(B, T - N)
        return w

    def forward(self, rays_o, rays_d, z, z_out, background_rgb, cos_anneal_ratio, skip_far=False, ray_grads=False, pending_merge=None,
                after_sdf=None, fuse_loss=None, before_heads=None, rest_normals=False, cos_anneal_dev=None, ray_grads_compact=False):
        r, w, B, N, T = self.r, self.w, self.B, self.N, self.T
        st = _stream()
        if ray_grads and skip_far and not ray_grads_compact:
            raise ValueError("ray gradients need every inside sample evaluated (skip_far=False)")
        self._ray_grads = bool(ray_grads)
        self._car_dev = cos_anneal_dev
        self._fwd_rays = (rays_o, rays_d)
        if ray_grads:
            self._ray_workspaces()
        for net in self.nets.values():
            net.img = net.module._images(join=before_heads is None)
        if self._ptr_key() != self._param_ptrs:
            raise RuntimeError("parameters were re-allocated after the training engine was built; rebuild it")
        sample_dist = 2.0 / r.n_samples
        O = r.n_outside
        self._fg_compact = bool(skip_far) and O > 0 and os.environ.get("VDN_FG_COMPACT", "1") != "0"
        self._color_fused = (self.precision == "bf16" and not self.dbc and not ray_grads and "c2" in self.nets["color"].img.blobs
                             and r.color_network.conf["d_out"] == 3 and os.environ.get("VDN_TRAIN_COLOR_FUSED", "0") == "1"
                             and not self._tail_wanted())
        from dpt_models.renderer import background_active, bg_compaction
        self._bg_compact = O > 0 and bg_compaction()
        fused_prep = self._bg_compact and os.environ.get("VDN_FUSED_PREP", "1") != "0"
        if pending_merge is not None and not fused_prep:
            new_z, M_old = pending_merge
            m = lib.VdnMergeArgs()
            m.z, m.new_z, m.z_out = z.data_ptr(), new_z.data_ptr(), z.data_ptr()
            m.B, m.M, m.K, m.ld, m.ld_out = B, M_old, N - M_old, z.stride(0), z.stride(0)
            lib.call("vdn_merge_sorted", m, st)
            pending_merge = None
        if O > 0 and not fused_prep:
            m = lib.VdnMergeArgs()
            m.z, m.new_z, m.z_out = z.data_ptr(), z_out.data_ptr(), w["z_feed"].data_ptr()
            m.B, m.M, m.K, m.ld, m.ld_out = B, N, O, z.stride(0), T
            lib.call("vdn_merge_sorted", m, st)
        if fused_prep:
            tp = lib.VdnTrainPrepArgs()
            tp.rays_o, tp.rays_d, tp.z, tp.z_out, tp.z_feed = (t.data_ptr() for t in (rays_o, rays_d, z, z_out, w["z_feed"]))
            tp.B, tp.N, tp.T, tp.z_ld, tp.sample_dist, tp.fg_radius = B, N, T, z.stride(0), sample_dist, 1.2
            if pending_merge is not None:
                tp.new_z, tp.M_old = pending_merge[0].data_ptr(), pending_merge[1]
            tp.dists, tp.mid_z, tp.bg_dists, tp.bg_mid = (w[k].data_ptr() for k in ("dists", "mid_z", "bg_dists", "bg_mid"))
            if self._fg_compact:
                tp.fg_active_idx, tp.fg_n_active, tp.fg_ray_counts = (t.data_ptr() for t in w["fg_active"])
            tp.bg_active_idx, tp.bg_n_active, tp.bg_ray_counts = (t.data_ptr() for t in w["bg_active"])
            lib.call("vdn_train_prep", tp, st)
            if fuse_loss is not None and fuse_loss.get("after_prep") is not None:
                fuse_loss["after_prep"](self)
        else:
            a = lib.VdnSectionArgs()
            a.z, a.dists, a.mid_z, a.sample_dist, a.B, a.n, a.ld = z.data_ptr(), w["dists"].data_ptr(), w["mid_z"].data_ptr(), sample_dist, B, N, z.stride(0)
            lib.call("vdn_sections", a, st)
            if self._fg_compact:
                fa = lib.VdnForegroundActiveArgs()
                fa.rays_o, fa.rays_d, fa.mid_z, fa.B, fa.N, fa.radius = rays_o.data_ptr(), rays_d.data_ptr(), w["mid_z"].data_ptr(), B, N, 1.2
                fa.active_idx, fa.n_active, fa.ray_counts = (t.data_ptr() for t in w["fg_active"])
                lib.call("vdn_foreground_active", fa, st)
        if not self._fg_compact:
            w["fg_active"][1].fill_(self.P)
        if O > 0:
            if not fused_prep:
                a = lib.VdnSectionArgs()
                a.z, a.dists, a.mid_z, a.sample_dist, a.B, a.n, a.ld = w["z_feed"].data_ptr(), w["bg_dists"].data_ptr(), w["bg_mid"].data_ptr(), sample_dist, B, T, T
                lib.call("vdn_sections", a, st)
            n = lib.VdnNerfArgs()
            n.blob = self.nets["nerf"].img.blobs["fwd"].data_ptr()
            n.rays_o, n.rays_d, n.z, n.n_per_ray, n.P = rays_o.data_ptr(), rays_d.data_ptr(), w["bg_mid"].data_ptr(), T, self.Q
            n.density, n.rgb = w["bg_density"].data_ptr(), w["bg_rgb"].data_ptr()
            n.feat = w["bg_feat"].data_ptr() if w["bg_feat"] is not None else None
            n.save_h, n.save_pe, n.save_feature, n.save_vpe, n.save_hv = (w[k].data_ptr() for k in ("nf_h", "nf_pe", "nf_feature", "nf_vpe", "nf_hv"))
            if self._bg_compact:
                if not fused_prep:
                    background_active(rays_o, rays_d, w["mid_z"], T, out=w["bg_active"])
                n.active_idx, n.n_active = w["bg_active"][0].data_ptr(), w["bg_active"][1].data_ptr()
            else:
                w["bg_active"][1].fill_(self.Q)
            self._fork()
            lib.call("vdn_nerf_mlp_fwd" + self.sfx, n, self._side_handle(st))
            if rest_normals and self._fg_compact:
                self._sdf_rest(rays_o, rays_d, self._side_handle(st))
            self._side_done()
        if self._color_fused and before_heads is not None:
            before_heads()
            before_heads = None
        self._sdf_forward(rays_o, rays_d)
        if after_sdf is not None:
            after_sdf(self)

        def rnet(net, out, save_h, small, d_out, module, stream=None):
            c = lib.VdnRenderNetArgs()
            c.blob = self.nets[net].img.blobs["fwd"].data_ptr()
            c.rays_o, c.rays_d, c.z, c.n_per_ray = rays_o.data_ptr(), rays_d.data_ptr(), w["mid_z"].data_ptr(), N
            c.normals, c.feat, c.out = w["normals"].data_ptr(), w["feat"].data_ptr(), out.data_ptr()
            c.save_h, c.save_small = save_h.data_ptr(), small.data_ptr()
            c.P, c.d_out, c.squeeze_out = self.P, d_out, int(module.squeeze_out)
            if net == "color" and self.dbc:
                c.extra, c.save_extra = w["vdn_out"].data_ptr(), w["col_extra"].data_ptr()
            lib.call("vdn_rendernet_fwd" + self.sfx, self._fg(c), st if stream is None else stream)
        if before_heads is not None:
            before_heads()
        vdn_beside = self.wdepth and self._side2 is not None and not self.dbc
        if self.wdepth:
            if vdn_beside:
                self._ev_fork2.record(lib.current_stream())
                self._side2.wait_event(self._ev_fork2)
                rnet("vdn", w["vdn_out"], w["vdn_h"], w["vdn_small"], 96, r.depth_network, stream=self._side2.cuda_stream)
                self._ev_join2.record(self._side2)
            else:
                rnet("vdn", w["vdn_out"], w["vdn_h"], w["vdn_small"], 96, r.depth_network)
        if not self._color_fused:
            rnet("color", w["col_out"], w["col_h"], w["col_small"], 3, r.color_network)
        if vdn_beside:
            lib.current_stream().wait_event(self._ev_join2)

        c = self._composite_common(lib.VdnCompositeArgs(), rays_o, rays_d, background_rgb, cos_anneal_ratio)
        c.weights, c.alpha_out, c.cdf, c.inside_sphere = w["weights"].data_ptr(), w["alpha"].data_ptr(), w["cdf"].data_ptr(), w["inside"].data_ptr()
        c.color_out, c.weight_sum, c.weight_max, c.s_val = w["color"].data_ptr(), w["wsum"].data_ptr(), w["wmax"].data_ptr(), w["s_val"].data_ptr()
        c.eik_partial, c.eik_out = w["eik_partial"].data_ptr(), w["eik"].data_ptr()
        if self.wdepth:
            c.feat_out = w["feat_out"].data_ptr()
        self._join()
        self._ctx = (rays_o, rays_d, background_rgb, cos_anneal_ratio, z)
        self._composite_bwd_done = False
        self._bwd_train = None
        if fuse_loss is not None and fuse_loss.get("before_composite") is not None:
            if not (fused_prep and self._fg_compact):
                raise RuntimeError("fuse_loss with a global foreground count needs the fused step preparation and the work lists")
            fuse_loss["before_composite"]()
        fg_count = lib.ptr(fuse_loss["fg_count"] if (fuse_loss is not None and fuse_loss.get("fg_count") is not None) else w["fg_active"][1])
        if fuse_loss is not None and self._fg_compact and self.wdepth and fuse_loss.get("gt_feats") is not None and not ray_grads:
            lib.call("vdn_composite_fwd_train", c, lib.ptr(fuse_loss["gt_feats"]), lib.ptr(fuse_loss["g_feats"]),
                     float(fuse_loss["depth_weight"]), float(fuse_loss["grad_scale"]), st)
            self._bwd_train = fuse_loss
        elif fuse_loss is not None and self._fg_compact and not self.wdepth and not ray_grads:
            cb = self._composite_bwd_args(None, None, None, None, None)
            self._fused_keep = (c, cb, fuse_loss)
            lib.call("vdn_composite_train", c, cb, lib.ptr(fuse_loss["true_rgb"]), lib.ptr(fuse_loss["g_color"]), fg_count,
                     float(fuse_loss["igr_weight"]), float(fuse_loss["grad_scale"]), st)
            self._composite_bwd_done = True
        else:
            lib.call("vdn_alpha_composite_fwd", c, st)
        self.generation = getattr(self, "generation", 0) + 1
        return w

    def _fg(self, args):
        if self._fg_compact:
            args.active_idx, args.n_active = self.w["fg_active"][0].data_ptr(), self.w["fg_active"][1].data_ptr()
        return args

    def _fork(self):
        if self._side is not None:
            self._ev_fork.record(lib.current_stream())
            self._side.wait_event(self._ev_fork)

    def _side_handle(self, main_handle):
        return main_handle if self._side is None else self._side.cuda_stream

    def _side_done(self):
        if self._side is not None:
            self._ev_join.record(self._side)
            self._pending = True

    def _join(self):
        if self._side is not None and self._pending:
            lib.current_stream().wait_event(self._ev_join)
            self._pending = False

    def _tail_wanted(self):
        tail_default = "1" if self._side is None else "0"
        return (self.precision == "bf16" and self._fg_compact and os.environ.get("VDN_SDF_TAIL", tail_default) != "0"
                and not getattr(self, "_ray_grads", False))

    def _sdf_rest(self, rays_o, rays_d, stream):
        w, N = self.w, self.N
        if "fg_rest" not in w:
            w["fg_rest"] = (torch.zeros(self.P, dtype=torch.int32, device=self.dev), torch.zeros(1, dtype=torch.int32, device=self.dev),
                            torch.zeros(self.B, dtype=torch.int32, device=self.dev))
        fa = lib.VdnForegroundActiveArgs()
        fa.rays_o, fa.rays_d, fa.mid_z, fa.B, fa.N, fa.radius = rays_o.data_ptr(), rays_d.data_ptr(), w["mid_z"].data_ptr(), self.B, N, 1.2
        fa.complement = 1
        fa.active_idx, fa.n_active, fa.ray_counts = (t.data_ptr() for t in w["fg_rest"])
        lib.call("vdn_foreground_active", fa, stream)
        s = lib.VdnSdfArgs()
        img = self.nets["sdf"].img
        s.blob = img.blobs["full"].data_ptr()
        s.rays_o, s.rays_d, s.z, s.n_per_ray, s.z_ld, s.sdf_ld = rays_o.data_ptr(), rays_d.data_ptr(), w["mid_z"].data_ptr(), N, N, N
        s.P, s.scale = self.P, float(self.r.sdf_network.scale)
        s.sdf, s.feat, s.normals = w["sdf"].data_ptr(), w["d_featvec"].data_ptr(), w["normals"].data_ptr()
        s.w8row = img.weff_view("lin8").data_ptr()
        if "S" in w:
            if "S_rest" not in w:
                w["S_rest"] = torch.empty_like(w["S"])
            s.S = w["S_rest"].data_ptr()
        s.active_idx, s.n_active = w["fg_rest"][0].data_ptr(), w["fg_rest"][1].data_ptr()
        lib.call("vdn_sdf_mlp_fwd" + self.sfx, 1, s, stream)

    def _sdf_forward(self, rays_o, rays_d):
        r, w, N = self.r, self.w, self.N
        s = lib.VdnSdfArgs()
        img = self.nets["sdf"].img
        s.blob = img.blobs["full"].data_ptr()
        s.rays_o, s.rays_d, s.z, s.n_per_ray, s.z_ld, s.sdf_ld = rays_o.data_ptr(), rays_d.data_ptr(), w["mid_z"].data_ptr(), N, N, N
        s.P, s.scale = self.P, float(r.sdf_network.scale)
        s.sdf, s.feat, s.normals = w["sdf"].data_ptr(), w["feat"].data_ptr(), w["normals"].data_ptr()
        if "S" in w:
            s.S = w["S"].data_ptr()
        s.w8row = img.weff_view("lin8").data_ptr()
        s.H, s.V, s.PE = w["H"].data_ptr(), w["V"].data_ptr(), w["PE"].data_ptr()
        if getattr(self, "_ray_grads", False):
            s.U_pe = w["U_pe"].data_ptr()
        tail = self._tail_wanted()
        fused = getattr(self, "_color_fused", False) and not tail
        if tail:
            row0 = int(os.environ.get("VDN_SDF_TAIL_ROW0", str(128 * torch.cuda.get_device_properties(self.dev).multi_processor_count)))
            tail = self.P > row0
            if tail:
                s.tail_row0, s.tail_max_rows = row0, int(os.environ.get("VDN_SDF_TAIL_MAX", "8192"))

        def launch():
            if fused:
                cimg = self.nets["color"].img
                lib.call("vdn_sdf_color_train_bf16", self._fg(s), lib.ptr(cimg.blobs["c2"]), int(r.color_network.squeeze_out),
                         lib.ptr(w["col_h"]), lib.ptr(w["col_small"]), lib.ptr(w["col_out"]), _stream())
                return
            lib.call("vdn_sdf_mlp_fwd" + self.sfx, 1, self._fg(s), _stream())
            if tail:
                lib.call("vdn_sdf_fwd_tail_bf16", s, _stream())
        probe = getattr(self, "sdf_probe", None)
        if probe is None:
            launch()
            return
        e0, e1 = torch.cuda.Event(enable_timing=True), torch.cuda.Event(enable_timing=True)
        e0.record()
        launch()
        e1.record()
        probe.append((e0, e1, w["fg_active"][1].clone() if self._fg_compact else None))

    def _dw_rows(self):
        n = {"bg": int(self.w["bg_active"][1].item()) if "bg_active" in self.w else 0, "fg": int(self.w["fg_active"][1].item())}
        tab = np.frombuffer(self.dw_table.cpu().numpy().tobytes(), dtype=lib.struct_dtype("VdnDwDesc"))
        return tab, [min(int(d["P"]), n[k]) for d, k in zip(tab, self.dw_list_kind)]

    def dw_bytes(self):
        esz = 4 if self.precision == "fp32" else 2
        total = 0
        tab, rows = self._dw_rows()
        for d, r in zip(tab, rows):
            segs = 2 if d["A2"] else 1
            total += segs * r * 32 * (int(d["m_tiles"]) + int(d["n_tiles"])) * esz
            total += int(d["splits"]) * int(d["m_tiles"]) * 32 * int(d["n_tiles"]) * 32 * 4
        return total

    def dw_flops(self):
        tab, rows = self._dw_rows()
        return sum(2.0 * (2 if d["A2"] else 1) * r * int(d["m_tiles"]) * 32 * int(d["n_tiles"]) * 32 for d, r in zip(tab, rows))

    def _launch_dw(self):
        lib.call("vdn_dw_gemm" + self.sfx, lib.ptr(self.dw_table), self.n_dw, self.dw_total_wgs, _stream())

    def _launch_dw_groups(self):
        for group in ("sdf", "rest"):
            if group in self.dw_groups:
                tab, n, wgs = self.dw_groups[group]
                lib.call("vdn_dw_gemm" + self.sfx, lib.ptr(tab), n, wgs, _stream())

    def side_weight_grads(self, group, after=None, gemm_event=None):
        if self._side is None:
            self.weight_grads(group, _stream())
            return None
        if after is not None:
            self._side.wait_event(after)
        elif group != "nerf":
            self._side.wait_event(self._ev_heads)
        self.weight_grads(group, self._side.cuda_stream, gemm_event, event_stream=self._side)
        self._pending = False
        return self._side

    def rest_weight_grads(self, after=None, gemm_event=None):
        if self._side is None:
            self.weight_grads("rest", _stream())
            return None
        if after is not None:
            self._side.wait_event(after)
        else:
            self._side.wait_event(self._ev_heads)
        self.weight_grads("rest", self._side.cuda_stream, gemm_event, event_stream=self._side)
        self._pending = False
        return self._side

    def weight_grads(self, group, stream, gemm_event=None, event_stream=None):
        if group in self.dw_groups:
            tab, n, wgs = self.dw_groups[group]
            lib.call("vdn_dw_gemm" + self.sfx, lib.ptr(tab), n, wgs, stream)
        if gemm_event is not None:
            gemm_event.record(event_stream if event_stream is not None else lib.current_stream())
        if group in self.fin_groups:
            tab, n, max_m, phase1 = self.fin_groups[group]
            lib.call("vdn_dw_finalize", lib.ptr(tab), n, max_m, 0, stream)
            if phase1:
                lib.call("vdn_dw_finalize", lib.ptr(tab), n, max_m, 1, stream)
        if group in self.wn_groups:
            tab, n, max_rows = self.wn_groups[group]
            lib.call("vdn_weightnorm_bwd", lib.ptr(tab), n, max_rows, stream)

    def _composite_common(self, c, rays_o, rays_d, background_rgb, cos_anneal_ratio):
        w, r = self.w, self.r
        c.rays_o, c.rays_d, c.sdf, c.normals = rays_o.data_ptr(), rays_d.data_ptr(), w["sdf"].data_ptr(), w["normals"].data_ptr()
        c.dists, c.mid_z, c.color = w["dists"].data_ptr(), w["mid_z"].data_ptr(), w["col_out"].data_ptr()
        c.variance = r.deviation_network.variance.data_ptr()
        if self.wdepth:
            c.feat, c.feat_ch = w["vdn_out"].data_ptr(), 96
        if r.n_outside > 0:
            c.bg_density, c.bg_rgb, c.bg_dists = w["bg_density"].data_ptr(), w["bg_rgb"].data_ptr(), w["bg_dists"].data_ptr()
            if self.wdepth:
                c.bg_feat = w["bg_feat"].data_ptr()
        if background_rgb is not None:
            c.background_rgb = background_rgb.data_ptr()
        c.cos_anneal_ratio = float(cos_anneal_ratio)
        if getattr(self, "_car_dev", None) is not None:
            c.cos_anneal_dev = self._car_dev.data_ptr()
        c.B, c.N, c.T = self.B, self.N, self.T
        return c

    def _composite_bwd_args(self, g_color, g_feat, g_weights, g_eik, g_cdf):
        r, w = self.r, self.w
        rays_o, rays_d, background_rgb, car, z = self._ctx
        c = self._composite_common(lib.VdnCompositeBwdArgs(), rays_o, rays_d, background_rgb, car)
        c.alpha, c.weights, c.eik = w["alpha"].data_ptr(), w["weights"].data_ptr(), w["eik"].data_ptr()
        c.g_cdf = g_cdf.data_ptr() if g_cdf is not None else None
        c.g_color = g_color.data_ptr() if g_color is not None else None
        c.g_feat = g_feat.data_ptr() if (g_feat is not None and self.wdepth) else None
        c.g_weights = g_weights.data_ptr() if g_weights is not None else None
        c.g_eik = g_eik.data_ptr() if g_eik is not None else None
        c.d_sdf, c.d_normals, c.d_color = w["d_sdf"].data_ptr(), w["d_normals"].data_ptr(), w["d_color"].data_ptr()
        if self.wdepth:
            c.d_feat = w["d_vdn"].data_ptr()
            c.feat_scratch = w["feat_scratch"].data_ptr()
            if g_feat is None:
                w["d_vdn"].zero_()
        if r.n_outside > 0:
            c.d_bg_density, c.d_bg_rgb = w["d_bg_density"].data_ptr(), w["d_bg_rgb"].data_ptr()
            if self.wdepth:
                c.d_bg_feat = w["d_bg_feat"].data_ptr()
                if g_feat is None:
                    w["d_bg_feat"].zero_()
        c.d_var_partial = w["d_var_partial"].data_ptr()
        if getattr(self, "_ray_grads", False):
            c.d_dists, c.d_dir_cos = w["d_dists"].data_ptr(), w["d_dir_cos"].data_ptr()
            if r.n_outside > 0:
                c.d_bg_dists = w["d_bg_dists"].data_ptr()
        self._bwd_args_keep = (g_color, g_feat, g_weights, g_eik, g_cdf)
        return c

    def backward(self, g_color, g_feat, g_weights, g_eik, g_cdf=None, g_gradients=None, defer_rest=False, gemm_event=None,
                 fork_event=None, heads_event=True):
        r, w, st = self.r, self.w, _stream()
        self._bwd_warm = True
        rays_o, rays_d, background_rgb, car, z = self._ctx
        keep = [t.contiguous() if t is not None else None for t in (g_color, g_feat, g_weights, g_eik, g_cdf, g_gradients)]
        g_color, g_feat, g_weights, g_eik, g_cdf, g_gradients = keep
        if (g_cdf is not None or g_gradients is not None) and self._fg_compact:
            raise ValueError("adjoints of cdf_fine / gradients need every inside sample evaluated (skip_far=False)")
        use_vdn = self.wdepth and g_feat is not None
        rg = getattr(self, "_ray_grads", False)
        if getattr(self, "_composite_bwd_done", False):
            self._composite_bwd_done = False
        elif getattr(self, "_bwd_train", None) is not None:
            fl, self._bwd_train = self._bwd_train, None
            c = self._composite_bwd_args(None, g_feat, None, None, None)
            lib.call("vdn_composite_bwd_train", c, lib.ptr(w["color"]), lib.ptr(fl["true_rgb"]), lib.ptr(fl["g_color"]),
                     lib.ptr(fl["fg_count"] if fl.get("fg_count") is not None else w["fg_active"][1]),
                     float(fl["igr_weight"]), float(fl["grad_scale"]), st)
        else:
            c = self._composite_bwd_args(g_color, g_feat, g_weights, g_eik, g_cdf)
            lib.call("vdn_alpha_composite_bwd", c, st)
        if g_gradients is not None:
            w["d_normals"].add_(g_gradients.reshape(self.P, 3))
        if r.n_outside > 0:
            nb = lib.VdnNerfBwdArgs()
            nb.blob = self.nets["nerf"].img.blobs["bwd"].data_ptr()
            nb.g_density, nb.g_rgb = w["d_bg_density"].data_ptr(), w["d_bg_rgb"].data_ptr()
            nb.g_feat = w["d_bg_feat"].data_ptr() if self.wdepth else None
            nb.save_h, nb.save_hv = w["nf_h"].data_ptr(), w["nf_hv"].data_ptr()
            nb.delta_o, nb.delta_v, nb.delta_head, nb.delta_h = (w[k].data_ptr() for k in ("nf_do", "nf_dv", "nf_dhead", "nf_dh"))
            nb.P = self.Q
            if self._bg_compact:
                nb.active_idx, nb.n_active = w["bg_active"][0].data_ptr(), w["bg_active"][1].data_ptr()
            if rg:
                w["d_bg_pts"].zero_()
                w["d_bg_dirs"].zero_()
                nb.rays_o, nb.rays_d, nb.z, nb.n_per_ray = rays_o.data_ptr(), rays_d.data_ptr(), w["bg_mid"].data_ptr(), self.T
                nb.d_pts, nb.d_dirs = w["d_bg_pts"].data_ptr(), w["d_bg_dirs"].data_ptr()
            if fork_event is not None and self._side is not None:
                self._side.wait_event(fork_event)
            else:
                self._fork()
            lib.call("vdn_nerf_mlp_bwd" + self.sfx, nb, self._side_handle(st))
            split_dw = (not defer_rest and self._side is not None and not rg and os.environ.get("VDN_BWD_SPLIT_DW", "1") != "0"
                        and all(k in self.dw_groups for k in ("sdf", "heads", "nerf")))
            if split_dw:
                self.weight_grads("nerf", self._side.cuda_stream)
            self._side_done()

        def rnet_bwd(net, g_out, out, save_h, dout, dh, d_out, module, accumulate):
            b = lib.VdnRenderNetBwdArgs()
            b.blob = self.nets[net].img.blobs["bwd"].data_ptr()
            b.g_out, b.out, b.save_h = g_out.data_ptr(), out.data_ptr(), save_h.data_ptr()
            b.delta_out, b.delta_h = dout.data_ptr(), dh.data_ptr()
            b.d_feat, b.d_normals = w["d_featvec"].data_ptr(), w["d_normals"].data_ptr()
            b.acc_feat, b.acc_normals = int(accumulate), 1
            b.P, b.d_out, b.squeeze_out = self.P, d_out, int(module.squeeze_out)
            if net == "color" and self.dbc:
                b.d_extra = w["d_vdn"].data_ptr()
            if rg:
                b.rays_d, b.n_per_ray, b.acc_pts = rays_d.data_ptr(), self.N, int(accumulate)
                b.d_pts, b.d_dirs = w["d_pts"].data_ptr(), w["d_dirs"].data_ptr()
            lib.call("vdn_rendernet_bwd" + self.sfx, self._fg(b), st)
        if rg and self._fg_compact:
            w["d_pts"].zero_()
            w["d_dirs"].zero_()
        rnet_bwd("color", w["d_color"], w["col_out"], w["col_h"], w["col_dout"], w["col_dh"], 3, r.color_network, False)
        if self.wdepth:
            rnet_bwd("vdn", w["d_vdn"], w["vdn_out"], w["vdn_h"], w["vdn_dout"], w["vdn_dh"], 96, r.depth_network, True)
        if defer_rest and self._side is not None and heads_event:
            self._ev_heads.record(lib.current_stream())

        rb = lib.VdnSdfRbarArgs()
        img = self.nets["sdf"].img
        rb.blob = img.blobs["full"].data_ptr()
        rb.rays_o, rb.rays_d, rb.z, rb.n_per_ray, rb.z_ld = rays_o.data_ptr(), rays_d.data_ptr(), w["mid_z"].data_ptr(), self.N, self.N
        rb.P, rb.scale = self.P, float(r.sdf_network.scale)
        s_from_h = 2 if self.precision == "bf16" else 0
        s_planes = w["H"] if s_from_h else w["S"]
        rb.g_normals, rb.S, rb.V, rb.UB, rb.EX = w["d_normals"].data_ptr(), s_planes.data_ptr(), w["V"].data_ptr(), w["UB"].data_ptr(), w["EX"].data_ptr()
        rb.s_from_h = s_from_h
        one_launch = self.precision == "bf16" and not rg and os.environ.get("VDN_SDF_BWD_SPLIT", "1") != "0"
        fb = lib.VdnSdfFbarArgs()
        fb.blob = img.blobs["fbar"].data_ptr()
        fb.g_sdf, fb.g_feat, fb.S, fb.EX, fb.AB = w["d_sdf"].data_ptr(), w["d_featvec"].data_ptr(), s_planes.data_ptr(), w["EX"].data_ptr(), w["AB"].data_ptr()
        fb.P, fb.scale, fb.s_from_h = self.P, float(r.sdf_network.scale), s_from_h
        if rg:
            fb.rays_o, fb.rays_d, fb.z, fb.n_per_ray, fb.z_ld = rays_o.data_ptr(), rays_d.data_ptr(), w["mid_z"].data_ptr(), self.N, self.N
            fb.g_normals, fb.U_pe, fb.acc_pts, fb.d_pts = w["d_normals"].data_ptr(), w["U_pe"].data_ptr(), 1, w["d_pts"].data_ptr()
        if not (one_launch and lib.try_call("vdn_sdf_bwd_split_bf16", self._fg(rb), self._fg(fb), st)):
            lib.call("vdn_sdf_bwd_rbar" + self.sfx, self._fg(rb), st)
            lib.call("vdn_sdf_bwd_fbar" + self.sfx, self._fg(fb), st)

        if defer_rest:
            if rg:
                raise ValueError("defer_rest is the Trainer's path: no ray gradients there")
            self.weight_grads("sdf", st, gemm_event)
            return self._grad_flat
        if r.n_outside > 0 and split_dw:
            self.weight_grads("sdf", st)
            self.weight_grads("heads", st)
            self._join()
        else:
            self._join()
            self._launch_dw()
            lib.call("vdn_dw_finalize", lib.ptr(self.fin_table), self.n_fin, self.fin_max_M, 0, st)
            if self.fin_has_phase1:
                lib.call("vdn_dw_finalize", lib.ptr(self.fin_table), self.n_fin, self.fin_max_M, 1, st)
            if self.n_wn:
                lib.call("vdn_weightnorm_bwd", lib.ptr(self.wn_table), self.n_wn, self.wn_max_rows, st)
        if rg:
            ra = lib.VdnRayAdjointArgs()
            ra.rays_d, ra.mid_z = rays_d.data_ptr(), w["mid_z"].data_ptr()
            ra.d_pts, ra.d_dirs, ra.d_dists, ra.d_dir_cos = (w[k].data_ptr() for k in ("d_pts", "d_dirs", "d_dists", "d_dir_cos"))
            ra.B, ra.N, ra.T = self.B, self.N, self.T
            if r.n_outside > 0:
                ra.bg_mid = w["bg_mid"].data_ptr()
                ra.d_bg_pts, ra.d_bg_dirs, ra.d_bg_dists, ra.d_z_out = (w[k].data_ptr() for k in ("d_bg_pts", "d_bg_dirs", "d_bg_dists", "d_z_out"))
            ra.d_rays_o, ra.d_rays_d, ra.d_z = w["d_rays_o"].data_ptr(), w["d_rays_d"].data_ptr(), w["d_z"].data_ptr()
            lib.call("vdn_ray_adjoint", ra, st)
        return self._grad_flat

    def outputs_clone(self):
        a = self._out_arena.clone()
        if self.__dict__.get("_out_strided") is None:
            self._out_strided = [(k, tuple(sh), tuple(torch.empty(sh, device="meta").stride()), o) for k, (o, sh) in self._out_slots.items()]
        st, base = a.untyped_storage(), a.storage_offset()
        return {k: torch.empty(0, dtype=torch.float32, device=a.device).set_(st, base + o, sh, sd) for k, sh, sd, o in self._out_strided}

    def param_grads(self, clone=True):
        if getattr(self, "join_hook", None) is not None:
            self.join_hook()
        if not clone:
            return [self.grad_views[id(p)] for p in self.params]
        if self.__dict__.get("_clone_slots") is None:
            slots, off = [], 0
            for p in self.params:
                slots.append((tuple(p.shape), tuple(self.grad_views[id(p)].stride()), off))
                off += (p.numel() + 63) // 64 * 64
            self._clone_slots, self._clone_total = slots, off
            self._grad_list = [self.grad_views[id(p)] for p in self.params]
        flat = torch.empty(self._clone_total, dtype=torch.float32, device=self._grad_flat.device)
        out = [flat.as_strided(sh, st, o) for sh, st, o in self._clone_slots]
        torch._foreach_copy_(out, self._grad_list)
        return out
```

Before: 406,200 rays/s.

## Save ReLU activation bitmasks in forward and use them in backward

The forward kernels for the NeRF and render MLPs now also write a bit-packed ReLU mask per hidden layer, one bit per unit. The backward kernels load these small masks once at the start and select gradients with them, instead of streaming the full bf16 saved activations per layer to test h>0. The goal is to cut global-memory reads in backward, which has to stay memory-bound. The cost is extra mask stores in the forward pass, more registers held for the mask words, and new template variants. It is enabled by default for bf16.

```diff
diff --git a/include/vdn_render.h b/include/vdn_render.h
--- a/include/vdn_render.h
+++ b/include/vdn_render.h
@@ -92,6 +92,7 @@
     const int32_t* n_active;
     const float* extra;
     void* save_extra;
+    void* save_mask;
 } VdnRenderNetArgs;
 int vdn_rendernet_fwd_f32(const VdnRenderNetArgs* args_host, void* stream);
 int vdn_rendernet_fwd_bf16(const VdnRenderNetArgs* args_host, void* stream);
@@ -115,6 +116,8 @@
     int32_t P;
     const int32_t* active_idx;
     const int32_t* n_active;
+    void* save_mask;
+    void* save_mask_v;
 } VdnNerfArgs;
 int vdn_nerf_mlp_fwd_f32(const VdnNerfArgs* args_host, void* stream);
 int vdn_nerf_mlp_fwd_bf16(const VdnNerfArgs* args_host, void* stream);
@@ -246,6 +249,7 @@
     float* d_pts;
     float* d_dirs;
     float* d_extra;
+    const void* mask;
 } VdnRenderNetBwdArgs;
 int vdn_rendernet_bwd_f32(const VdnRenderNetBwdArgs* args_host, void* stream);
 int vdn_rendernet_bwd_bf16(const VdnRenderNetBwdArgs* args_host, void* stream);
@@ -268,6 +272,8 @@
     int32_t n_per_ray;
     float* d_pts;
     float* d_dirs;
+    const void* mask;
+    const void* mask_v;
 } VdnNerfBwdArgs;
 int vdn_nerf_mlp_bwd_f32(const VdnNerfBwdArgs* args_host, void* stream);
 int vdn_nerf_mlp_bwd_bf16(const VdnNerfBwdArgs* args_host, void* stream);
diff --git a/vdn-nerf_amd/csrc/k_nerf_bwd.h b/vdn-nerf_amd/csrc/k_nerf_bwd.h
--- a/vdn-nerf_amd/csrc/k_nerf_bwd.h
+++ b/vdn-nerf_amd/csrc/k_nerf_bwd.h
@@ -5,7 +5,7 @@
 
 namespace vdn {
 
-template <class P, bool DPT, bool EXPL>
+template <class P, bool DPT, bool EXPL, bool MASK = false>
 __global__ __launch_bounds__(P::kWaves * 64, P::kMinWavesPerEU) void nerf_bwd_kernel(NerfBwdArgs a, NerfInputGradArgs in) {
     using ST = typename P::store_t;
     constexpr int kSlot = P::stride(9);
@@ -31,6 +31,14 @@
     ST* delta_v = reinterpret_cast<ST*>(a.delta_v);
     ST* delta_head = reinterpret_cast<ST*>(a.delta_head);
     ST* delta_h = reinterpret_cast<ST*>(a.delta_h);
+    unsigned mk[MASK ? 34 : 1];
+    if constexpr (MASK) {
+        const unsigned char* m = static_cast<const unsigned char*>(a.mask);
+        const long MS = BF16::mask_plane(a.P, 256);
+#pragma unroll
+        for (int l = 0; l < 8; ++l) BF16::load_mask<4>(m + l * MS, p, h, mk + 4 * l);
+        BF16::load_mask<2>(static_cast<const unsigned char*>(a.mask_v), p, h, mk + 32);
+    }
 
     float x4[4] = {0.0f, 0.0f, 0.0f, 0.0f}, dir[3] = {0.0f, 0.0f, 0.0f}, pw[3] = {0.0f, 0.0f, 0.0f}, nrm = 1.0f;
     float dx4[4] = {0.0f, 0.0f, 0.0f, 0.0f}, ddir[3] = {0.0f, 0.0f, 0.0f};
@@ -81,11 +89,26 @@
             P::store_tile(dst, p, ld, nt, h, o, ok);
         };
     };
+    auto bit_store = [&](auto& D, ST* dst, int ld, int w0) VDN_INL {
+        return [&D, &mk, dst, ld, w0, p, ok, h](int nt, const f32x16& acc, int) VDN_INL {
+            const f32x16 o = BF16::mask_select(mk + w0, nt, acc);
+            D.set(nt, o);
+            P::store_tile(dst, p, ld, nt, h, o, ok);
+        };
+    };
+    auto hidden = [&](auto kt_c, auto& In, auto& D, int l) VDN_INL {
+        constexpr int KT = decltype(kt_c)::value;
+        if constexpr (MASK) dense<P, KT, 8, false>(ws, In, 0, NoPre{}, bit_store(D, delta_h + l * PS, 256, 4 * l), P::kTileOps);
+        else dense<P, KT, 8, false, kBwdPrefetch>(ws, In, 0, ldH(l), mask_store(D, delta_h + l * PS, 256), P::kTileOps, P::kTileOps);
+    };
+    using K8 = std::integral_constant<int, 8>;
     ws.all_issue = __any(ok);
+    if constexpr (MASK) BF16::mask_landed(mk);
     warm_l2_wait();
     ws.start();
-    dense<P, KO, 4, false>(ws, X, 0, [&](int nt) VDN_INL { return P::load_tile(save_hv, p, 128, nt, h); },
-                               mask_store(Y, delta_v, 128), 4);
+    if constexpr (MASK) dense<P, KO, 4, false>(ws, X, 0, NoPre{}, bit_store(Y, delta_v, 128, 32), P::kTileOps);
+    else dense<P, KO, 4, false>(ws, X, 0, [&](int nt) VDN_INL { return P::load_tile(save_hv, p, 128, nt, h); },
+                                    mask_store(Y, delta_v, 128), 4);
     dense<P, 4, 9, false>(ws, Y, 0, NoPre{}, [&](int nt, const f32x16& acc, int) VDN_INL {
         if (nt < 8) {
             X.set(nt, acc);
@@ -100,16 +123,23 @@
         X.set(8, t16);
         P::store_tile(delta_head, p, 288, 8, h, t16, ok);
     }
-    dense<P, 9, 8, false, kBwdPrefetch>(ws, X, 0, ldH(7), mask_store(Y, delta_h + 7 * PS, 256), P::kTileOps, P::kTileOps);
-    dense<P, 8, 8, false, kBwdPrefetch>(ws, Y, 0, ldH(6), mask_store(X, delta_h + 6 * PS, 256), P::kTileOps, P::kTileOps);
-    dense<P, 8, 8, false, kBwdPrefetch>(ws, X, 0, ldH(5), mask_store(Y, delta_h + 5 * PS, 256), P::kTileOps, P::kTileOps);
+    hidden(std::integral_constant<int, 9>{}, X, Y, 7);
+    hidden(K8{}, Y, X, 6);
+    hidden(K8{}, X, Y, 5);
     dense<P, 8, 11, false>(ws, Y, 0,
-        [&](int nt) VDN_INL { return nt >= 3 ? P::load_tile(save_h + 4 * PS, p, 256, nt - 3, h) : f32x16{}; },
-        [&](int nt, const f32x16& acc, const f32x16& hv) VDN_INL {
+        [&](int nt) VDN_INL {
+            if constexpr (MASK) return 0;
+            else return nt >= 3 ? P::load_tile(save_h + 4 * PS, p, 256, nt - 3, h) : f32x16{};
+        },
+        [&](int nt, const f32x16& acc, const auto& hv) VDN_INL {
             if (nt >= 3) {
                 f32x16 o;
-#pragma unroll
-                for (int t = 0; t < 16; ++t) o[t] = hv[t] > 0.0f ? acc[t] : 0.0f;
+                if constexpr (MASK) {
+                    o = BF16::mask_select(mk + 16, nt - 3, acc);
+                } else {
+#pragma unroll
+                    for (int t = 0; t < 16; ++t) o[t] = hv[t] > 0.0f ? acc[t] : 0.0f;
+                }
                 X.set(nt - 3, o);
                 P::store_tile(delta_h + 4 * PS, p, 256, nt - 3, h, o, ok);
             } else if (want_pts) {
@@ -118,10 +148,10 @@
                 else pe_adjoint_tile<4, 10, 2, P::kAccurateTrig>(acc, h, x4, dx4);
             }
         });
-    dense<P, 8, 8, false, kBwdPrefetch>(ws, X, 0, ldH(3), mask_store(Y, delta_h + 3 * PS, 256), P::kTileOps, P::kTileOps);
-    dense<P, 8, 8, false, kBwdPrefetch>(ws, Y, 0, ldH(2), mask_store(X, delta_h + 2 * PS, 256), P::kTileOps, P::kTileOps);
-    dense<P, 8, 8, false, kBwdPrefetch>(ws, X, 0, ldH(1), mask_store(Y, delta_h + 1 * PS, 256), P::kTileOps, P::kTileOps);
-    dense<P, 8, 8, false, kBwdPrefetch>(ws, Y, 0, ldH(0), mask_store(X, delta_h + 0 * PS, 256), P::kTileOps, P::kTileOps);
+    hidden(K8{}, X, Y, 3);
+    hidden(K8{}, Y, X, 2);
+    hidden(K8{}, X, Y, 1);
+    hidden(K8{}, Y, X, 0);
     if (want_pts) {
         dense<P, 8, 3, false>(ws, X, 0, NoPre{}, [&](int nt, const f32x16& acc, int) VDN_INL {
             if (nt == 0) pe_adjoint_tile<4, 10, 0, P::kAccurateTrig>(acc, h, x4, dx4);
@@ -158,6 +188,20 @@
     const int ppw = P::kWaves * 32;
     const int grid = (args->P + ppw - 1) / ppw;
     const size_t lds = 3 * P::stride(9);
+    if (args->mask != nullptr || args->mask_v != nullptr) {
+        if constexpr (std::is_same<P, BF16>::value && !EXPL) {
+            if (args->mask == nullptr || args->mask_v == nullptr) return -5;
+            static bool once_m = (allow_big_lds(nerf_bwd_kernel<P, false, false, true>, lds), allow_big_lds(nerf_bwd_kernel<P, true, false, true>, lds), true);
+            (void)once_m;
+            if (args->g_feat != nullptr)
+                hipLaunchKernelGGL((nerf_bwd_kernel<P, true, false, true>), dim3(grid), dim3(P::kWaves * 64), lds, stream, *args, in);
+            else
+                hipLaunchKernelGGL((nerf_bwd_kernel<P, false, false, true>), dim3(grid), dim3(P::kWaves * 64), lds, stream, *args, in);
+            return (int)hipGetLastError();
+        } else {
+            return -5;
+        }
+    }
     static bool once = (allow_big_lds(nerf_bwd_kernel<P, false, EXPL>, lds), allow_big_lds(nerf_bwd_kernel<P, true, EXPL>, lds), true);
     (void)once;
     if (args->g_feat != nullptr)
diff --git a/vdn-nerf_amd/csrc/k_nerf_fwd.h b/vdn-nerf_amd/csrc/k_nerf_fwd.h
--- a/vdn-nerf_amd/csrc/k_nerf_fwd.h
+++ b/vdn-nerf_amd/csrc/k_nerf_fwd.h
@@ -115,6 +115,7 @@
     if (args == nullptr || args->P <= 0 || !args->blob || !args->density || !args->rgb || args->n_per_ray <= 0) return -1;
     if (!args->pts4 && (!args->rays_o || !args->rays_d || !args->z)) return -1;
     if (!args->dirs && !args->rays_d) return -1;
+    if (args->save_mask || args->save_mask_v) return -2;
     const int ppw = P::kWaves * 32;
     const int grid = (args->P + ppw - 1) / ppw;
     const size_t lds = 3 * P::stride(11);
diff --git a/vdn-nerf_amd/csrc/k_nerf_fwd2.h b/vdn-nerf_amd/csrc/k_nerf_fwd2.h
--- a/vdn-nerf_amd/csrc/k_nerf_fwd2.h
+++ b/vdn-nerf_amd/csrc/k_nerf_fwd2.h
@@ -4,7 +4,7 @@
 
 namespace vdn {
 
-template <bool DPT, bool SAVE>
+template <bool DPT, bool SAVE, bool MASK = false>
 struct NerfFwdProg {
     static constexpr int total = 64 + 9 + 4 + (DPT ? 4 : 1);
     static constexpr int kt(int c) {
@@ -21,10 +21,10 @@
     static constexpr bool drained(int c) { return c == 39; }
     static constexpr int stores(int c) {
         if (!SAVE || c < 0 || c >= total) return 0;
-        if (c < 64) return BF16::kTileOps;
+        if (c < 64) return BF16::kTileOps + (MASK && c % 8 == 7 ? 1 : 0);
         if (c < 72) return BF16::kTileOps;
         if (c < 73) return 0;
-        if (c < 77) return BF16::kTileOps;
+        if (c < 77) return BF16::kTileOps + (MASK && c == 76 ? 1 : 0);
         return 0;
     }
 };
@@ -32,12 +32,13 @@
 #ifndef VDN_NERF_FWD_ST_MODE
 #define VDN_NERF_FWD_ST_MODE VDN_PLANE_ST_MODE
 #endif
-template <bool DPT, bool SAVE>
+template <bool DPT, bool SAVE, bool MASK = false>
 __global__ __launch_bounds__(256, 2) void nerf_fwd2_kernel(NerfArgs a) {
+    static_assert(SAVE || !MASK, "masks are training saves");
     constexpr int kSt = VDN_NERF_FWD_ST_MODE;
     using P = BF16;
     using ST = unsigned short;
-    using PG = NerfFwdProg<DPT, SAVE>;
+    using PG = NerfFwdProg<DPT, SAVE, MASK>;
     constexpr int kSlot = P::stride(11);
     extern __shared__ __attribute__((aligned(16))) char smem[];
     flow::Pipe<4, kSlot, 3, 2> pp;
@@ -93,32 +94,46 @@
 #pragma unroll
         for (int i = 0; i < 6; ++i) pe_keep[i] = X.r[i];
     }
-    auto relu_into = [&](auto& D, int t0, ST* save, int ld) VDN_INL {
-        return [&D, t0, save, ld, q, h](int nt, const f32x16& acc, int) VDN_INL {
+    unsigned mk[4];
+    auto relu_into = [&](auto& D, int t0, ST* save, int ld, unsigned char* msave = nullptr) VDN_INL {
+        return [&D, &mk, t0, save, ld, msave, q, h](int nt, const f32x16& acc, int) VDN_INL {
             f32x16 o;
 #pragma unroll
             for (int t = 0; t < 16; ++t) o[t] = relu0(acc[t]);
             D.set(t0 + nt, o);
             if constexpr (SAVE) P::template store_tile<kSt>(save, q, ld, nt, h, o, true);
+            if constexpr (MASK) {
+                const unsigned b = P::relu_bits(o);
+                if (nt & 1) mk[nt >> 1] |= b << 16;
+                else mk[nt >> 1] = b;
+                if (ld == 256 && nt == 7) P::template store_mask<4, kSt>(msave, q, h, mk, true);
+                if (ld == 128 && nt == 3) {
+                    const unsigned m2[2] = {mk[0], mk[1]};
+                    P::template store_mask<2, kSt>(msave, q, h, m2, true);
+                }
+            }
         };
     };
     auto sv = [&](int l) VDN_INL { return save_h + l * PS; };
+    unsigned char* const save_mask = static_cast<unsigned char*>(a.save_mask);
+    const long MS = P::mask_plane(a.P, 256);
+    auto sm = [&](int l) VDN_INL { return MASK ? save_mask + l * MS : nullptr; };
     warm_l2_wait();
     pp.template start<PG>();
     auto f0 = flow::flow_begin();
-    auto f1 = flow::dense2<PG, 8>(f0, pp, X, flow::NoLoad{}, relu_into(Y, 0, sv(0), 256));
-    auto f2 = flow::dense2<PG, 8>(f1, pp, Y, flow::NoLoad{}, relu_into(X, 0, sv(1), 256));
-    auto f3 = flow::dense2<PG, 8>(f2, pp, X, flow::NoLoad{}, relu_into(Y, 0, sv(2), 256));
-    auto f4 = flow::dense2<PG, 8>(f3, pp, Y, flow::NoLoad{}, relu_into(X, 0, sv(3), 256));
-    auto f5 = flow::dense2<PG, 8>(f4, pp, X, flow::NoLoad{}, relu_into(Y, 0, sv(4), 256));
+    auto f1 = flow::dense2<PG, 8>(f0, pp, X, flow::NoLoad{}, relu_into(Y, 0, sv(0), 256, sm(0)));
+    auto f2 = flow::dense2<PG, 8>(f1, pp, Y, flow::NoLoad{}, relu_into(X, 0, sv(1), 256, sm(1)));
+    auto f3 = flow::dense2<PG, 8>(f2, pp, X, flow::NoLoad{}, relu_into(Y, 0, sv(2), 256, sm(2)));
+    auto f4 = flow::dense2<PG, 8>(f3, pp, Y, flow::NoLoad{}, relu_into(X, 0, sv(3), 256, sm(3)));
+    auto f5 = flow::dense2<PG, 8>(f4, pp, X, flow::NoLoad{}, relu_into(Y, 0, sv(4), 256, sm(4)));
     auto f5d = flow::flow_drain(f5);
 #pragma unroll
     for (int kt = 0; kt < 8; ++kt) X.copy_tile(3 + kt, Y, kt);
 #pragma unroll
     for (int i = 0; i < 6; ++i) X.r[i] = pe_keep[i];
-    auto f6 = flow::dense2<PG, 8>(f5d, pp, X, flow::NoLoad{}, relu_into(Y, 0, sv(5), 256));
-    auto f7 = flow::dense2<PG, 8>(f6, pp, Y, flow::NoLoad{}, relu_into(X, 0, sv(6), 256));
-    auto f8 = flow::dense2<PG, 8>(f7, pp, X, flow::NoLoad{}, relu_into(Y, 0, sv(7), 256));
+    auto f6 = flow::dense2<PG, 8>(f5d, pp, X, flow::NoLoad{}, relu_into(Y, 0, sv(5), 256, sm(5)));
+    auto f7 = flow::dense2<PG, 8>(f6, pp, Y, flow::NoLoad{}, relu_into(X, 0, sv(6), 256, sm(6)));
+    auto f8 = flow::dense2<PG, 8>(f7, pp, X, flow::NoLoad{}, relu_into(Y, 0, sv(7), 256, sm(7)));
     auto f9 = flow::dense2<PG, 9>(f8, pp, Y, flow::NoLoad{}, [&](int nt, const f32x16& acc, int) VDN_INL {
         if (nt < 8) {
             X.set(nt, acc);
@@ -138,7 +153,8 @@
             if (a.save_vpe != nullptr) P::template store_tile<kSt>(reinterpret_cast<ST*>(a.save_vpe), q, 32, 0, h, t16, true);
         }
     }
-    auto f10 = flow::dense2<PG, 4, false>(f9, pp, X, flow::NoLoad{}, relu_into(Y, 0, reinterpret_cast<ST*>(a.save_hv), 128));
+    auto f10 = flow::dense2<PG, 4, false>(f9, pp, X, flow::NoLoad{}, relu_into(Y, 0, reinterpret_cast<ST*>(a.save_hv), 128,
+                                                                             static_cast<unsigned char*>(a.save_mask_v)));
     auto f11 = flow::dense2<PG, DPT ? 4 : 1>(f10, pp, Y, flow::NoLoad{}, [&](int nt, const f32x16& acc, int) VDN_INL {
         if (nt == 0) {
             if (ok && h == 0) {
@@ -160,15 +176,18 @@
     if (!args->dirs && !args->rays_d) return -1;
     const bool save = args->save_h != nullptr;
     if (save && (!args->save_hv || !args->save_feature)) return -1;
+    const bool mask = args->save_mask != nullptr;
+    if (mask != (args->save_mask_v != nullptr) || (mask && !save)) return -2;
     const int grid = (args->P + 127) / 128;
     const size_t lds = 3 * BF16::stride(11);
     static bool once = (allow_big_lds(nerf_fwd2_kernel<false, false>, lds), allow_big_lds(nerf_fwd2_kernel<true, false>, lds),
-                        allow_big_lds(nerf_fwd2_kernel<false, true>, lds), allow_big_lds(nerf_fwd2_kernel<true, true>, lds), true);
+                        allow_big_lds(nerf_fwd2_kernel<false, true>, lds), allow_big_lds(nerf_fwd2_kernel<true, true>, lds),
+                        allow_big_lds(nerf_fwd2_kernel<false, true, true>, lds), allow_big_lds(nerf_fwd2_kernel<true, true, true>, lds), true);
     (void)once;
     const bool dpt = args->feat != nullptr;
-#define VDN_L(D, S) hipLaunchKernelGGL((nerf_fwd2_kernel<D, S>), dim3(grid), dim3(256), lds, stream, *args)
-    if (dpt) { if (save) VDN_L(true, true); else VDN_L(true, false); }
-    else { if (save) VDN_L(false, true); else VDN_L(false, false); }
+#define VDN_L(D, S, M) hipLaunchKernelGGL((nerf_fwd2_kernel<D, S, M>), dim3(grid), dim3(256), lds, stream, *args)
+    if (dpt) { if (mask) VDN_L(true, true, true); else if (save) VDN_L(true, true, false); else VDN_L(true, false, false); }
+    else { if (mask) VDN_L(false, true, true); else if (save) VDN_L(false, true, false); else VDN_L(false, false, false); }
 #undef VDN_L
     return (int)hipGetLastError();
 }
diff --git a/vdn-nerf_amd/csrc/k_render_bwd.h b/vdn-nerf_amd/csrc/k_render_bwd.h
--- a/vdn-nerf_amd/csrc/k_render_bwd.h
+++ b/vdn-nerf_amd/csrc/k_render_bwd.h
@@ -5,7 +5,7 @@
 
 namespace vdn {
 
-template <class P, int NT_OUT, int EX = 0>
+template <class P, int NT_OUT, int EX = 0, bool MASK = false>
 __global__ __launch_bounds__(P::kWaves * 64, P::kMinWavesPerEU) void rendernet_bwd_kernel(RenderNetBwdArgs a) {
     using ST = typename P::store_t;
     constexpr int kSlot = P::stride(8);
@@ -24,6 +24,13 @@
     ST* delta_h = reinterpret_cast<ST*>(a.delta_h);
     ST* delta_out = reinterpret_cast<ST*>(a.delta_out);
     ST* d_feat = reinterpret_cast<ST*>(a.d_feat);
+    unsigned mk[MASK ? 16 : 1];
+    if constexpr (MASK) {
+        const unsigned char* m = static_cast<const unsigned char*>(a.mask);
+        const long MS = BF16::mask_plane(a.P, 256);
+#pragma unroll
+        for (int l = 0; l < 4; ++l) BF16::load_mask<4>(m + l * MS, p, h, mk + 4 * l);
+    }
 
     typename P::template Act<8> X, Y;
     if constexpr (NT_OUT == 1) {
@@ -61,13 +68,28 @@
             P::store_tile(delta_h + l * PS, p, 256, nt, h, o, ok);
         };
     };
+    auto bit_store = [&](auto& D, int l) VDN_INL {
+        return [&D, &mk, l, delta_h, PS, p, ok, h](int nt, const f32x16& acc, int) VDN_INL {
+            const f32x16 o = BF16::mask_select(mk + 4 * l, nt, acc);
+            D.set(nt, o);
+            P::store_tile(delta_h + l * PS, p, 256, nt, h, o, ok);
+        };
+    };
     ws.all_issue = __any(ok);
+    if constexpr (MASK) BF16::mask_landed(mk);
     warm_l2_wait();
     ws.start();
-    dense<P, NT_OUT, 8, false, kBwdPrefetch>(ws, X, 0, ldH(3), mask_store(Y, 3), P::kTileOps, P::kTileOps);
-    dense<P, 8, 8, false, kBwdPrefetch>(ws, Y, 0, ldH(2), mask_store(X, 2), P::kTileOps, P::kTileOps);
-    dense<P, 8, 8, false, kBwdPrefetch>(ws, X, 0, ldH(1), mask_store(Y, 1), P::kTileOps, P::kTileOps);
-    dense<P, 8, 8, false, kBwdPrefetch>(ws, Y, 0, ldH(0), mask_store(X, 0), P::kTileOps, P::kTileOps);
+    if constexpr (MASK) {
+        dense<P, NT_OUT, 8, false>(ws, X, 0, NoPre{}, bit_store(Y, 3), P::kTileOps);
+        dense<P, 8, 8, false>(ws, Y, 0, NoPre{}, bit_store(X, 2), P::kTileOps);
+        dense<P, 8, 8, false>(ws, X, 0, NoPre{}, bit_store(Y, 1), P::kTileOps);
+        dense<P, 8, 8, false>(ws, Y, 0, NoPre{}, bit_store(X, 0), P::kTileOps);
+    } else {
+        dense<P, NT_OUT, 8, false, kBwdPrefetch>(ws, X, 0, ldH(3), mask_store(Y, 3), P::kTileOps, P::kTileOps);
+        dense<P, 8, 8, false, kBwdPrefetch>(ws, Y, 0, ldH(2), mask_store(X, 2), P::kTileOps, P::kTileOps);
+        dense<P, 8, 8, false, kBwdPrefetch>(ws, X, 0, ldH(1), mask_store(Y, 1), P::kTileOps, P::kTileOps);
+        dense<P, 8, 8, false, kBwdPrefetch>(ws, Y, 0, ldH(0), mask_store(X, 0), P::kTileOps, P::kTileOps);
+    }
     f32x16 SM[2];
     dense<P, 8, 10 + EX, false>(ws, X, 0, NoPre{}, [&](int nt, const f32x16& acc, int) VDN_INL {
         if (nt >= 10) {
@@ -129,6 +151,24 @@
     const int ppw = P::kWaves * 32;
     const int grid = (args->P + ppw - 1) / ppw;
     const size_t lds = 3 * P::stride(8);
+    if (args->mask != nullptr) {
+        if constexpr (std::is_same<P, BF16>::value) {
+            static bool once_m = (allow_big_lds(rendernet_bwd_kernel<P, 1, 0, true>, lds), allow_big_lds(rendernet_bwd_kernel<P, 3, 0, true>, lds),
+                                  allow_big_lds(rendernet_bwd_kernel<P, 1, 3, true>, lds), true);
+            (void)once_m;
+            if (args->d_extra != nullptr) {
+                if (args->d_out == 96) return -4;
+                hipLaunchKernelGGL((rendernet_bwd_kernel<P, 1, 3, true>), dim3(grid), dim3(P::kWaves * 64), lds, stream, *args);
+            } else if (args->d_out == 96) {
+                hipLaunchKernelGGL((rendernet_bwd_kernel<P, 3, 0, true>), dim3(grid), dim3(P::kWaves * 64), lds, stream, *args);
+            } else {
+                hipLaunchKernelGGL((rendernet_bwd_kernel<P, 1, 0, true>), dim3(grid), dim3(P::kWaves * 64), lds, stream, *args);
+            }
+            return (int)hipGetLastError();
+        } else {
+            return -5;
+        }
+    }
     static bool once = (allow_big_lds(rendernet_bwd_kernel<P, 1>, lds), allow_big_lds(rendernet_bwd_kernel<P, 3>, lds),
                         allow_big_lds(rendernet_bwd_kernel<P, 1, 3>, lds), true);
     (void)once;
diff --git a/vdn-nerf_amd/csrc/k_render_fwd.h b/vdn-nerf_amd/csrc/k_render_fwd.h
--- a/vdn-nerf_amd/csrc/k_render_fwd.h
+++ b/vdn-nerf_amd/csrc/k_render_fwd.h
@@ -58,13 +58,24 @@
             if (save_small != nullptr) P::store_tile(save_small, p, 64, kt, h, t16, ok);
         }
     }
+    unsigned char* const save_mask = static_cast<unsigned char*>(a.save_mask);
+    const long MS = P::plane(a.P, 32);
+    unsigned mk[4];
     auto relu_into = [&](auto& D, int l) VDN_INL {
-        return [&D, l, save_h, PS, p, ok, h](int nt, const f32x16& acc, int) VDN_INL {
+        return [&D, &mk, l, save_h, save_mask, MS, PS, p, ok, h](int nt, const f32x16& acc, int) VDN_INL {
             f32x16 o;
 #pragma unroll
             for (int t = 0; t < 16; ++t) o[t] = relu0(acc[t]);
             D.set(nt, o);
             if (save_h != nullptr) P::store_tile(save_h + l * PS, p, 256, nt, h, o, ok);
+            if constexpr (std::is_same<P, BF16>::value) {
+                if (save_mask != nullptr) {
+                    const unsigned b = BF16::relu_bits(o);
+                    if (nt & 1) mk[nt >> 1] |= b << 16;
+                    else mk[nt >> 1] = b;
+                    if (nt == 7) BF16::store_mask<4>(save_mask + l * MS, p, h, mk, ok);
+                }
+            }
         };
     };
     const int est = save_h != nullptr ? P::kTileOps : 0;
@@ -102,6 +113,7 @@
     if (!args->pts && (!args->rays_o || !args->rays_d || !args->z)) return -1;
     if (!args->dirs && !args->rays_d) return -1;
     if (!(args->d_out == 96 || (args->d_out >= 1 && args->d_out <= 4))) return -2;
+    if (args->save_mask && (!args->save_h || !std::is_same<P, BF16>::value)) return -4;
     const int ppw = P::kWaves * 32;
     const int grid = (args->P + ppw - 1) / ppw;
     if (args->extra != nullptr) {
diff --git a/vdn-nerf_amd/csrc/mlp_engine.h b/vdn-nerf_amd/csrc/mlp_engine.h
--- a/vdn-nerf_amd/csrc/mlp_engine.h
+++ b/vdn-nerf_amd/csrc/mlp_engine.h
@@ -354,6 +354,68 @@
     }
     static VDN_DEV f32x16 load_tile(const unsigned short* base, long row, int ld, int tile, int h) {
         return unpack(load_raw(base, row, ld, tile, h));
+    }
+
+    static VDN_DEV long mask_plane(long P, int ld) { return rows(P) * (ld / 8); }
+    static VDN_DEV unsigned relu_bits(const f32x16& v) {
+        unsigned m = 0;
+#pragma unroll
+        for (int j = 0; j < 8; ++j) {
+            const unsigned u = pack_bf16x2(v[2 * j], v[2 * j + 1]);
+            m |= (bf16_lo(u) > 0.0f ? 1u : 0u) << (2 * j);
+            m |= (bf16_hi(u) > 0.0f ? 1u : 0u) << (2 * j + 1);
+        }
+        return m;
+    }
+    template <int NW>
+    static VDN_DEV unsigned char* mask_ptr(unsigned char* base, long row, int h) {
+        return base + (row >> 5) * (64L * 4 * NW) + h * (32 * 4 * NW) + (row & 31) * (4 * NW);
+    }
+    template <int NW, int MODE = VDN_PLANE_ST_MODE>
+    static VDN_DEV void store_mask(unsigned char* base, long row, int h, const unsigned (&m)[NW], bool ok) {
+        static_assert(NW == 2 || NW == 4, "mask: 128- or 256-wide layers");
+        if (!ok) return;
+        unsigned char* p = mask_ptr<NW>(base, row, h);
+        if constexpr (NW == 4) {
+            typedef unsigned mk_u32x4 __attribute__((ext_vector_type(4)));
+            const mk_u32x4 ov = {m[0], m[1], m[2], m[3]};
+            if constexpr (MODE == 1) asm volatile("global_store_dwordx4 %0, %1, off sc1\n\ts_nop 1" ::"v"(p), "v"(ov) : "memory");
+            else if constexpr (MODE == 2) asm volatile("global_store_dwordx4 %0, %1, off nt\n\ts_nop 1" ::"v"(p), "v"(ov) : "memory");
+            else if constexpr (MODE == 3) asm volatile("global_store_dwordx4 %0, %1, off sc1 nt\n\ts_nop 1" ::"v"(p), "v"(ov) : "memory");
+            else if constexpr (MODE == 4) { asm volatile("" ::"v"(p), "v"(ov)); }
+            else *reinterpret_cast<uint4*>(p) = make_uint4(m[0], m[1], m[2], m[3]);
+        } else {
+            typedef unsigned mk_u32x2 __attribute__((ext_vector_type(2)));
+            const mk_u32x2 ov = {m[0], m[1]};
+            if constexpr (MODE == 1) asm volatile("global_store_dwordx2 %0, %1, off sc1\n\ts_nop 1" ::"v"(p), "v"(ov) : "memory");
+            else if constexpr (MODE == 2) asm volatile("global_store_dwordx2 %0, %1, off nt\n\ts_nop 1" ::"v"(p), "v"(ov) : "memory");
+            else if constexpr (MODE == 3) asm volatile("global_store_dwordx2 %0, %1, off sc1 nt\n\ts_nop 1" ::"v"(p), "v"(ov) : "memory");
+            else if constexpr (MODE == 4) { asm volatile("" ::"v"(p), "v"(ov)); }
+            else *reinterpret_cast<uint2*>(p) = make_uint2(m[0], m[1]);
+        }
+    }
+    template <int NW>
+    static VDN_DEV void load_mask(const unsigned char* base, long row, int h, unsigned* m) {
+        const unsigned char* p = mask_ptr<NW>(const_cast<unsigned char*>(base), row, h);
+        if constexpr (NW == 4) {
+            const uint4 v = *reinterpret_cast<const uint4*>(p);
+            m[0] = v.x; m[1] = v.y; m[2] = v.z; m[3] = v.w;
+        } else {
+            const uint2 v = *reinterpret_cast<const uint2*>(p);
+            m[0] = v.x; m[1] = v.y;
+        }
+    }
+    template <int N>
+    static VDN_DEV void mask_landed(unsigned (&m)[N]) {
+#pragma unroll
+        for (int i = 0; i < N; ++i) asm volatile("" : "+v"(m[i]));
+    }
+    static VDN_DEV f32x16 mask_select(const unsigned* m, int nt, const f32x16& acc) {
+        const unsigned b = m[nt >> 1] >> (16 * (nt & 1));
+        f32x16 o;
+#pragma unroll
+        for (int t = 0; t < 16; ++t) o[t] = ((b >> t) & 1u) ? acc[t] : 0.0f;
+        return o;
     }
 };
 
diff --git a/vdn-nerf_amd/vdn_hip/layout.py b/vdn-nerf_amd/vdn_hip/layout.py
--- a/vdn-nerf_amd/vdn_hip/layout.py
+++ b/vdn-nerf_amd/vdn_hip/layout.py
@@ -28,3 +28,11 @@
         return col0
     assert col0 % 32 == 0
     return (col0 // 32) * 1024
+
+
+def mask_from_plane(buf, P, ld):
+    Pp = pad32(P)
+    b = buf.reshape(-1)[:Pp * ld // 8].view(Pp // 32, 2, 32, ld // 16).long()
+    bits = (b.unsqueeze(-1) >> torch.arange(8, device=b.device)) & 1
+    bits = bits.reshape(Pp // 32, 2, 32, ld // 32, 2, 2, 4)
+    return bits.permute(0, 2, 3, 4, 5, 1, 6).reshape(Pp, ld)[:P].bool()
diff --git a/vdn-nerf_amd/vdn_hip/train.py b/vdn-nerf_amd/vdn_hip/train.py
--- a/vdn-nerf_amd/vdn_hip/train.py
+++ b/vdn-nerf_amd/vdn_hip/train.py
@@ -264,6 +264,11 @@
             w["vdn_out"], w["vdn_h"], w["vdn_small"] = fz(P, 96), fs(4, Pp, 256), fs(Pp, 64)
         if self.dbc:
             w["col_extra"] = fs(Pp, 96)
+        self.relu_mask = self.precision == "bf16" and os.environ.get("VDN_RELU_MASK", "1") != "0"
+        fm = lambda *shape: torch.empty(*shape, dtype=torch.uint8, device=dev) if self.relu_mask else None
+        w["col_mask"] = fm(4, Pp * 32)
+        if self.wdepth:
+            w["vdn_mask"] = fm(4, Pp * 32)
         if O > 0:
             w["z_feed"], w["bg_dists"], w["bg_mid"] = f(B, T), f(B, T), out("bg_mid")
             w["bg_density"], w["bg_rgb"] = torch.zeros(Q, device=dev), torch.zeros(Q, 3, device=dev)
@@ -271,6 +276,7 @@
             w["bg_active"] = (torch.zeros(Q, dtype=torch.int32, device=dev), torch.zeros(1, dtype=torch.int32, device=dev),
                               torch.zeros(B, dtype=torch.int32, device=dev))
             w["nf_h"], w["nf_pe"], w["nf_feature"], w["nf_vpe"], w["nf_hv"] = fs(8, Qp, 256), fs(Qp, 96), fs(Qp, 256), fs(Qp, 32), fs(Qp, 128)
+            w["nf_mask"], w["nf_mask_v"] = fm(8, Qp * 32), fm(Qp * 16)
         w["weights"], w["alpha"], w["cdf"], w["inside"] = out("weights"), f(B, T), out("cdf"), out("inside")
         w["color"], w["wsum"], w["wmax"], w["s_val"] = out("color"), out("wsum"), out("wmax"), out("s_val")
         w["eik_partial"], w["eik"] = f(B, 2), out("eik")
@@ -467,6 +473,8 @@
             n.density, n.rgb = w["bg_density"].data_ptr(), w["bg_rgb"].data_ptr()
             n.feat = w["bg_feat"].data_ptr() if w["bg_feat"] is not None else None
             n.save_h, n.save_pe, n.save_feature, n.save_vpe, n.save_hv = (w[k].data_ptr() for k in ("nf_h", "nf_pe", "nf_feature", "nf_vpe", "nf_hv"))
+            if self.relu_mask:
+                n.save_mask, n.save_mask_v = w["nf_mask"].data_ptr(), w["nf_mask_v"].data_ptr()
             if self._bg_compact:
                 if not fused_prep:
                     background_active(rays_o, rays_d, w["mid_z"], T, out=w["bg_active"])
@@ -491,6 +499,8 @@
             c.rays_o, c.rays_d, c.z, c.n_per_ray = rays_o.data_ptr(), rays_d.data_ptr(), w["mid_z"].data_ptr(), N
             c.normals, c.feat, c.out = w["normals"].data_ptr(), w["feat"].data_ptr(), out.data_ptr()
             c.save_h, c.save_small = save_h.data_ptr(), small.data_ptr()
+            if self.relu_mask:
+                c.save_mask = w[net[:3] + "_mask"].data_ptr()
             c.P, c.d_out, c.squeeze_out = self.P, d_out, int(module.squeeze_out)
             if net == "color" and self.dbc:
                 c.extra, c.save_extra = w["vdn_out"].data_ptr(), w["col_extra"].data_ptr()
@@ -780,6 +790,8 @@
             nb.g_density, nb.g_rgb = w["d_bg_density"].data_ptr(), w["d_bg_rgb"].data_ptr()
             nb.g_feat = w["d_bg_feat"].data_ptr() if self.wdepth else None
             nb.save_h, nb.save_hv = w["nf_h"].data_ptr(), w["nf_hv"].data_ptr()
+            if self.relu_mask:
+                nb.mask, nb.mask_v = w["nf_mask"].data_ptr(), w["nf_mask_v"].data_ptr()
             nb.delta_o, nb.delta_v, nb.delta_head, nb.delta_h = (w[k].data_ptr() for k in ("nf_do", "nf_dv", "nf_dhead", "nf_dh"))
             nb.P = self.Q
             if self._bg_compact:
@@ -804,6 +816,8 @@
             b = lib.VdnRenderNetBwdArgs()
             b.blob = self.nets[net].img.blobs["bwd"].data_ptr()
             b.g_out, b.out, b.save_h = g_out.data_ptr(), out.data_ptr(), save_h.data_ptr()
+            if self.relu_mask and not (net == "color" and self._color_fused):
+                b.mask = w[net[:3] + "_mask"].data_ptr()
             b.delta_out, b.delta_h = dout.data_ptr(), dh.data_ptr()
             b.d_feat, b.d_normals = w["d_featvec"].data_ptr(), w["d_normals"].data_ptr()
             b.acc_feat, b.acc_normals = int(accumulate), 1
```

New measurement: 419,900 rays/s (median of 6 runs). 1.03x the previous value.
